# knights-lab/BURST

Hardware: AMD Instinct MI355X
Metric: aligned reads/sec (node), 100-bp synthetic reads @0.98 id vs RefSeq stand-in .edx/.acx (DB15), -m BEST; 1 GPU (higher is better)
Workload: dtype u32 bit-vectors (u8 edit distances)

## Files before the change

burst_amd/csrc/bhip_align.hip:

```cpp
#include "bhip_handle.h"
#include "bhip_pf_select.h"

__global__ void k_hit_count(const BhipHit *__restrict__ hits, uint32_t n, const uint32_t *__restrict__ n_dev, uint32_t *__restrict__ cnt, uint32_t *__restrict__ rank) {
	if (n_dev) n = *n_dev < n ? *n_dev : n;
	for (uint32_t i = blockIdx.x * blockDim.x + threadIdx.x; i < n; i += gridDim.x * blockDim.x) rank[i] = atomicAdd(&cnt[hits[i].q], 1u);
}
__global__ void k_hit_scatter(const BhipHit *__restrict__ in, uint32_t n, const uint32_t *__restrict__ n_dev, const uint32_t *__restrict__ off, const uint32_t *__restrict__ rank,
                              BhipHit *__restrict__ out, const uint32_t *__restrict__ qmap) {
	if (n_dev) n = *n_dev < n ? *n_dev : n;
	for (uint32_t i = blockIdx.x * blockDim.x + threadIdx.x; i < n; i += gridDim.x * blockDim.x) {
		BhipHit h = in[i];
		const uint32_t dst = off[h.q] + rank[i];
		if (qmap) h.q = qmap[h.q];
		out[dst] = h;
	}
}
__global__ void k_junk_adjust_raw(BhipRawHit *__restrict__ raw, const uint32_t *__restrict__ n_raw_dev, uint32_t raw_cap, const uint8_t *__restrict__ nx) {
	uint32_t n = *n_raw_dev;
	if (n > raw_cap) n = raw_cap;
	for (uint32_t i = blockIdx.x * blockDim.x + threadIdx.x; i < n; i += gridDim.x * blockDim.x) { const uint32_t x = nx[raw[i].q]; raw[i].ed += x; raw[i].m += x; }
}
__global__ void k_junk_adjust_best(uint32_t *__restrict__ best, const uint8_t *__restrict__ nx_six, uint32_t s0, uint32_t s1) {
	for (uint32_t s = s0 + blockIdx.x * blockDim.x + threadIdx.x; s < s1; s += gridDim.x * blockDim.x)
		if (nx_six[s] && best[s] != 0xFFFFFFFFu) best[s] += nx_six[s];
// ... 325 lines not shown
	HIPCHK(hipEventRecord(ev[SPAN_START], st));
	const uint64_t full = (n_thr + 255) / 256;
	const uint32_t grid = (uint32_t)(ahead && h->opt_seed_ahead_blocks > 0 ? std::min<uint64_t>(full, (uint64_t)h->n_cu * (uint64_t)h->opt_seed_ahead_blocks) : full);
	hipLaunchKernelGGL(k_seed_ranges, dim3(grid), dim3(256), 0, st,
		junk ? S->qcodes_s.as<uint8_t>() : S->qcodes.as<uint8_t>(), junk ? S->qoff_s.as<uint64_t>() : S->qoff.as<uint64_t>(), d_qlist, n_list,
		h->acx_view(), h->K, S->plan.as<uint32_t>(), W16, L->ranges_c[cls].as<uint2>(), L->hdr_c[cls].as<uint2>(),
		junk ? S->qpack_s.as<uint32_t>() : S->qpack.as<uint32_t>(), (S->st_maxlen + 7) / 8, junk ? S->qemac_s.as<uint16_t>() : S->qemac.as<uint16_t>(), qm.as<uint4>(), S->st_has_six ? S->qsix.as<uint32_t>() : nullptr,
		seed_min_need_for(h, mean_words, W16), (uint32_t)h->opt_seed_drop_len, h->alt);
	HIPCHK(hipGetLastError());
	HIPCHK(hipEventRecord(ev[SPAN_DONE], st));
	L->qmeta_seq[S->seq & 1][cls] = S->seq + 1;
	L->seeded_ok[cls] = true; L->seeded_seq[cls] = S->seq; L->seeded_n[cls] = n_list; L->seeded_W16[cls] = W16;
	return 0;
}

static bhip_pf_kernel_t pf_kernel(const BhipPfChoice &c, int big) {
	if (c.legacy) return bhip_legacy_pf_kernel ? bhip_legacy_pf_kernel(c.kind, big ? 11 : c.htb, big ? 4 : c.rb, c.cw_mode, big) : nullptr;
	if (c.kind == BHIP_PF_CQ) return c.cw_mode == 0 ? (big ? k_prefilter_cq<0, 1> : k_prefilter_cq<0, 0>) : (big ? k_prefilter_cq<1, 1> : k_prefilter_cq<1, 0>);
	return big ? k_prefilter_cw<2, 1> : k_prefilter_cw<2, 0>;
}

static int launch_prefilter_mask(Handle *h, Lane *L, hipStream_t st, int cls, const uint32_t *d_qlist, uint32_t n_list, uint32_t maxwords, uint32_t *n_tasks_dev,
                                 uint32_t *n_cand_dev, Counters *dc, int algo, int prune) {
	int rc;
	PfOverflow ov;
	if ((rc = ov.begin(L, dc, st, n_list, true))) return rc;
	const uint32_t W16 = seed_row_words(maxwords);
	const double mean_words = n_list ? (double)L->seed_words[cls] / (double)n_list : (double)maxwords;
	if (!(L->seeded_ok[cls] && L->seeded_seq[cls] == h->cur->seq && L->seeded_n[cls] == n_list && L->seeded_W16[cls] == W16))
		if ((rc = launch_seed(h, L, st, h->cur, cls, d_qlist, n_list, maxwords, mean_words))) return rc;
	const BhipPfChoice c = bhip_pf_choose(algo, h->opt_pf_cw, h->opt_pf_table, h->opt_pf_rb, W16, mean_words * h->acx_wmean);
	const bool filter = c.kind != BHIP_PF_MASK, cw = c.kind == BHIP_PF_CW || c.kind == BHIP_PF_CQ;
	const bhip_pf_kernel_t fp = filter ? pf_kernel(c, 0) : nullptr, fp2 = filter && c.two_pass ? pf_kernel(c, 1) : nullptr;
	if (filter && (!fp || (c.two_pass && !fp2)))
		return fail(BHIP_E_ARG, "option prefilter_cw = %d selects a superseded prefilter kernel that is not part of libburst_hip.so (tests: libburst_hip_legacy.so is loaded first)", h->opt_pf_cw);
	hipFuncAttributes fa;
	const void *fn = filter ? (const void *)fp : c.htb == 9 ? (const void *)k_prefilter_mask<9> : c.htb == 10 ? (const void *)k_prefilter_mask<10> : (const void *)k_prefilter_mask<11>;
	const uint32_t fit = std::min<uint32_t>(cw ? 32u : 12u, blocks_per_cu(fn, 64u, 0, &fa));
	if (getenv("BHIP_DEBUG")) {
		if (cw) fprintf(stderr, "[bhip] prefilter kernel: %s, slot mode %d, %zu B LDS, %d VGPRs -> %u blocks per CU\n", c.kind == BHIP_PF_CQ ? "four queries per wave, streams by the whole wave" : "one query per wave", c.cw_mode, fa.sharedSizeBytes, fa.numRegs, fit);
		else fprintf(stderr, "[bhip] prefilter kernel: table 2^%d, %d record blocks in registers, %zu B LDS, %d VGPRs -> %u blocks per CU\n", c.htb, c.rb, fa.sharedSizeBytes, fa.numRegs, fit);
	}
	const uint32_t waves = h->opt_pf_waves ? std::min<uint32_t>((uint32_t)h->opt_pf_waves, fit) : fit;
	const uint32_t grid = std::min<uint32_t>(c.kind == BHIP_PF_CW ? n_list : (n_list + 3) / 4, (uint32_t)h->n_cu * waves);
	HIPCHK(hipEventRecord(L->ev_pf[cls][PF_HASH_START], st));
	const uint32_t *fb_dense = ov.fb1, *n_fb_dense = ov.n_fb1;
	if (filter) {
		auto launch = [&](bhip_pf_kernel_t k, uint32_t g, uint32_t *fb, uint32_t *n_fb, const uint32_t *sel, const uint32_t *n_sel) {
			hipLaunchKernelGGL(k, dim3(g), dim3(64), 0, st, L->ranges_c[cls].as<uint2>(), L->hdr_c[cls].as<uint2>(), W16, n_list,
				h->acx_view().rec, h->bad.as<uint32_t>(), h->n_bad,
				h->clump_len.as<uint32_t>(), h->tot_refs, L->tasks.as<uint2>(), n_tasks_dev, (uint32_t)L->task_cap, &dc->ent_read,
				fb, n_fb, &dc->unit_sum, &dc->col_sum, &dc->qlen_sum, &dc->surv_sum,
				L->tasks2.as<uint2>(), &dc->n_tasks2_cls[cls], prune, sel, n_sel, c.kind == BHIP_PF_CF ? h->opt_pf_bytes : 0);
		};
		launch(fp, grid, ov.fb1, ov.n_fb1, nullptr, nullptr);
		if (c.two_pass) {
			HIPCHK(hipGetLastError());
			const uint32_t g2 = (uint32_t)h->n_cu * (c.kind == BHIP_PF_CQ ? std::min<uint32_t>(4u, blocks_per_cu((const void *)fp2, 64u, 0)) : 1u);
			launch(fp2, g2, ov.fb2, ov.n_fb2, ov.fb1, ov.n_fb1);
			fb_dense = ov.fb2; n_fb_dense = ov.n_fb2;
		}
	} else {
		dispatch_int(HtbList{}, c.htb, [&](auto htb) {
			hipLaunchKernelGGL(k_prefilter_mask<decltype(htb)::value>, dim3(grid), dim3(64), 0, st, L->ranges_c[cls].as<uint2>(), L->hdr_c[cls].as<uint2>(), W16, n_list,
				h->acx_view().rec, h->bad.as<uint32_t>(), h->n_bad,
				h->clump_len.as<uint32_t>(), h->tot_refs, L->tasks.as<uint2>(), n_tasks_dev, (uint32_t)L->task_cap, &dc->ent_read,
				ov.fb1, ov.n_fb1, &dc->unit_sum, &dc->col_sum, &dc->qlen_sum, L->cand.as<uint2>(), n_cand_dev, (uint32_t)L->cand_cap);
		});
	}
	HIPCHK(hipGetLastError());
	HIPCHK(hipEventRecord(L->ev_pf[cls][PF_HASH_DONE], st));
	++L->pf_launches;
	L->pf_algo_used = c.kind;
	return launch_dense_fallback(h, L, st, d_qlist, n_list, h->bad.as<uint32_t>(), h->n_bad, L->cand.as<uint2>(), nullptr, n_cand_dev, (uint32_t)L->cand_cap, dc, fb_dense, n_fb_dense);
}

static int lane_reserve_work(Lane *L) {
	int rc;
	if ((rc = L->cand.reserve(L->cand_cap * sizeof(uint2))) || (rc = L->raw.reserve(L->raw_cap * sizeof(BhipRawHit))) || (rc = L->wide.reserve(L->raw_cap * sizeof(uint32_t))) ||
	    (rc = L->rs_lists.reserve(L->raw_cap * sizeof(uint32_t) * 10)) || (rc = L->scratch.reserve(L->scratch_cap * sizeof(uint32_t))) || (rc = L->wins.reserve(L->win_cap * sizeof(BhipWin))) ||
	    (rc = L->tasks.reserve(L->task_cap * sizeof(uint2))) || (rc = L->tasks2.reserve(L->task_cap * sizeof(uint2))) || (rc = L->tasks2k.reserve(L->task_cap * sizeof(uint2))) ||
	    (rc = L->wins2.reserve(L->win_cap * sizeof(BhipWin)))) return rc;
	return 0;
}
extern "C" int bhip_reserve(void *handle, uint32_t n_entries, uint32_t max_len) { return bhip_reserve_symbols(handle, n_entries, max_len, 0); }
extern "C" int bhip_reserve_symbols(void *handle, uint32_t n_entries, uint32_t max_len, uint64_t total_symbols) {
	Handle *h = (Handle *)handle;
	if (!h) return fail(BHIP_E_ARG, "null handle");
	if (!n_entries) return BHIP_OK;
	if (!max_len || max_len > BHIP_MAX_QLEN) max_len = BHIP_MAX_QLEN;
	HIPCHK(hipSetDevice(h->device));
	int rc;
	if (getenv("BHIP_DEBUG")) { size_t f_ = 0, t_ = 0; if (hipMemGetInfo(&f_, &t_) == hipSuccess) fprintf(stderr, "[bhip] reserve for %u entries of up to %u symbols: %.2f GB of the device's %.2f free\n", n_entries, max_len, f_ / 1e9, t_ / 1e9); }
	const size_t n = n_entries, nb = total_symbols ? (size_t)std::min<uint64_t>(total_symbols + 64, (uint64_t)n * max_len) : n * max_len, qw = (max_len + 7) / 8;
	const size_t cw = (size_t)class_words(class_of_len(max_len), max_len);
	const size_t peq_words = total_symbols ? std::min<size_t>(n * cw, 2 * (nb / 32 + n)) : n * cw;
	for (StageSlot &S : h->slots) {
		if ((rc = slot_init(&S))) return rc;
		if ((rc = S.qcodes4.reserve(nb / 2 + 128)) || (rc = S.qcodes.reserve(nb + 128)) || (rc = S.qoff.reserve((n + 1) * 8)) || (rc = S.qemac.reserve((n + 1) * 2)) ||
		    (rc = S.qsix.reserve((n + 1) * 4)) || (rc = S.qrc.reserve(n + 1)) || (rc = S.qflags.reserve(n + 1)) || (rc = S.qmap.reserve((n + 1) * 4)) ||
		    (rc = S.off_raw.reserve((n + 8) * 8)) || (rc = S.plan.reserve(n * 4 + 16)) || (rc = S.qpack.reserve(n * qw * 4 + 64)) || (rc = S.key.reserve(n + 16)) ||
		    (rc = S.key_sorted.reserve(n + 16)) || (rc = S.idx.reserve(n * 4 + 16)) || (rc = S.idx_sorted.reserve(n * 4 + 16))) return rc;
		size_t tb = 0;
		HIPCHK(hipcub::DeviceRadixSort::SortPairs(nullptr, tb, S.key.as<uint8_t>(), S.key_sorted.as<uint8_t>(), S.idx.as<uint32_t>(), S.idx_sorted.as<uint32_t>(), (int)n, 0, 8, h->stage_stream));
		if ((rc = S.sort_tmp.reserve(tb + 16))) return rc;
	}
	if (getenv("BHIP_DEBUG")) { size_t f_ = 0, t_ = 0; if (hipMemGetInfo(&f_, &t_) == hipSuccess) fprintf(stderr, "[bhip] ... staging slots reserved: %.2f GB free\n", f_ / 1e9); }
	if ((rc = ensure_lanes(h, 1))) return rc;
	Lane *L = h->lanes[0];
	lane_capacity_floor(h, L, n);
	const int cls = class_of_len(max_len);
	if ((rc = lane_reserve_work(L)) || (rc = L->peq.reserve(peq_words * 16 * 4)) || (rc = L->peqp.reserve(n * 16 * 6 * 4)) ||
	    (rc = L->peq_alt.reserve(peq_words * 16 * 4)) || (rc = L->peqp_alt.reserve(n * 16 * 6 * 4)) ||
	    (rc = L->fb_list.reserve(n * 8 + 64)) || (rc = L->ranges_c[cls].reserve(n * 16 * 8 + 16)) || (rc = L->hdr_c[cls].reserve(n * 8 + 16))) return rc;
	if (h->n_order) { if ((rc = h->best_key.reserve((n + 1) * 8)) || (rc = h->sort_idx.reserve(std::max<size_t>((size_t)h->out_cap, n + 1) * 4))) return rc; if (!h->nsel_pinned) HIPCHK(hipHostMalloc((void **)&h->nsel_pinned, 64, hipHostMallocDefault)); }
	if ((rc = h->best.reserve((n + 1) * 4)) || (rc = h->out.reserve(h->out_cap * sizeof(BhipHit))) || (rc = h->shared_ctr.reserve(sizeof(SharedCtr))) ||
	    (rc = h->sort_idx.reserve(h->out_cap * 4)) || (rc = h->sort_keys.reserve((n + 1) * 4)) || (rc = h->sort_keys2.reserve((n + 1) * 4)) ||
	    (rc = h->out_sorted.reserve(h->out_cap * sizeof(BhipHit))) || (rc = h->out_sorted2.reserve(h->out_cap * sizeof(BhipHit)))) return rc;
	{
		size_t tb = 0;
		HIPCHK(hipcub::DeviceScan::ExclusiveSum(nullptr, tb, h->sort_keys.as<uint32_t>(), h->sort_keys2.as<uint32_t>(), (int)(n + 1), h->stream));
		if ((rc = h->sort_tmp.reserve(tb))) return rc;
	}
	if (getenv("BHIP_DEBUG")) { size_t f_ = 0, t_ = 0; if (hipMemGetInfo(&f_, &t_) == hipSuccess) fprintf(stderr, "[bhip] ... lane and record buffers reserved: %.2f GB free\n", f_ / 1e9); }
	if (!h->copy_stream) { HIPCHK(hipStreamCreateWithFlags(&h->copy_stream, hipStreamNonBlocking)); HIPCHK(hipEventCreateWithFlags(&h->ev_sorted, hipEventDisableTiming));
		for (auto &e : h->ev_copied) HIPCHK(hipEventCreateWithFlags(&e, hipEventDisableTiming)); }
	{
		const uint32_t nw = std::min<uint32_t>(n_entries, 1u << 17), len = std::min<uint32_t>(max_len, 100u);
		const size_t nb_w = (size_t)nw * len + 16;
		uint8_t *pin = nullptr;
		const size_t bytes = nb_w + nb_w / 2 + 16 + ((size_t)nw + 1) * 8 + (size_t)nw * 2 + 64 + (size_t)nw * 4 * sizeof(BhipHit);
		HIPCHK(hipHostMalloc((void **)&pin, bytes, hipHostMallocPortable));
		uint8_t *codes = pin, *codes4 = pin + nb_w;
		uint64_t *off = (uint64_t *)(pin + ((nb_w + nb_w / 2 + 16 + 7) & ~(size_t)7));
		uint16_t *emac = (uint16_t *)(off + nw + 1);
		BhipHit *hbuf = (BhipHit *)(((uintptr_t)(emac + nw) + 63) & ~(uintptr_t)63);
		uint64_t x = 88172645463325252ull;
		for (size_t i = 0; i < nb_w; ++i) { x ^= x << 13; x ^= x >> 7; x ^= x << 17; codes[i] = (uint8_t)(1 + (x & 3)); }
		for (size_t i = 0; i < nb_w / 2; ++i) codes4[i] = (uint8_t)(codes[2 * i] | codes[2 * i + 1] << 4);
		for (uint32_t i = 0; i <= nw; ++i) off[i] = (uint64_t)i * len;
		for (uint32_t i = 0; i < nw; ++i) emac[i] = (uint16_t)(len / 40);
		BhipQuerySpan sp;
		memset(&sp, 0, sizeof sp);
		sp.codes = codes; sp.codes4 = codes4; sp.off = off; sp.emac = emac; sp.n = nw;
		uint64_t n_out = 0;
		const int async = h->opt_async_d2h;
		h->opt_async_d2h = 1;
		for (StageSlot &S : h->slots) { S.state = 0; S.st_valid = false; }
		rc = 0;
		for (int rep = 0; rep < 4 && !rc; ++rep) {
			rc = bhip_stage_spans(h, &sp, 1, nw, len);
			if (!rc) rc = bhip_align_staged(h, 0, hbuf, (uint64_t)nw * 4, &n_out);
		}
		(void)bhip_sync_hits(h);
		{
			const size_t big = std::min<size_t>(64u << 20, std::min(h->out_sorted.cap, h->out_sorted2.cap));
			void *tmp = nullptr;
			if (big && hipHostMalloc(&tmp, 2 * big, hipHostMallocPortable) == hipSuccess) {
				(void)hipMemcpyAsync(tmp, h->out_sorted.p, big, hipMemcpyDeviceToHost, h->copy_stream);
				(void)hipMemcpyAsync((char *)tmp + big, h->out_sorted2.p, big, hipMemcpyDeviceToHost, h->copy_stream);
				(void)hipMemcpyAsync(tmp, h->out_sorted.p, big, hipMemcpyDeviceToHost, h->copy_stream);
				(void)hipStreamSynchronize(h->copy_stream);
				(void)hipMemcpyAsync(h->out_sorted.p, tmp, big, hipMemcpyHostToDevice, h->stage_stream);
				(void)hipMemcpyAsync(h->out_sorted2.p, (char *)tmp + big, big, hipMemcpyHostToDevice, h->stage_stream);
				(void)hipMemcpyAsync(h->out_sorted.p, tmp, big, hipMemcpyHostToDevice, h->stage_stream);
				(void)hipStreamSynchronize(h->stage_stream);
				const size_t piece = big / 16;
				if (piece) {
					for (int i = 0; i < 12; ++i) (void)hipMemcpyAsync((char *)h->out_sorted.p + (size_t)i * piece, (char *)tmp + (size_t)i * piece, piece, hipMemcpyHostToDevice, h->stage_stream);
					(void)hipMemcpyAsync((char *)tmp + big, h->out_sorted2.p, big, hipMemcpyDeviceToHost, h->copy_stream);
					(void)hipStreamSynchronize(h->copy_stream);
					(void)hipStreamSynchronize(h->stage_stream);
				}
				(void)hipHostFree(tmp);
			}
			(void)hipGetLastError();
		}
		h->opt_async_d2h = async;
		for (StageSlot &S : h->slots) { S.state = 0; S.st_valid = false; S.spans.clear(); }
		h->res_valid = false;
		(void)hipHostFree(pin);
		if (rc) return rc;
	}
	return BHIP_OK;
}
enum { STEP_REDO = 1 };
struct BatchCall {
	StageSlot *slot = nullptr;
	int mode = 0;
	int all_hits = 0;
	bool sel_best = false;
	BhipHit *hits = nullptr; uint64_t cap = 0; uint64_t *n_hits = nullptr;
	uint32_t n_q = 0, n_shared = 0, nl = 0;
	uint32_t band_rows = 0, qw = 0, rw = 0;
	SharedCtr hsc = {};
	uint32_t n_deliver = 0;
	bool sorted_ahead = false; int o_ahead = 0;
	size_t tmp_bytes = 0;
	std::chrono::steady_clock::time_point t0; double t_host[4] = {0, 0, 0, 0};
	void mark(int i) { t_host[i] = std::chrono::duration<double, std::milli>(std::chrono::steady_clock::now() - t0).count(); }
};

static int enqueue_class(Handle *h, Lane *L, int cls, int all_hits) {
	int rc;
	hipStream_t pf = h->pf_stream, sw = h->sweep_stream, po = h->post_stream;
	Counters *dc = L->counters.as<Counters>();
	const uint32_t n_pf = L->npf[cls], n_ex = L->nex[cls], n_list = n_pf + n_ex;
	const uint32_t grid_my = (uint32_t)h->n_cu * (uint32_t)h->opt_sweep_blocks;
	const uint32_t grid_task = (uint32_t)h->n_cu * 4u * (uint32_t)h->opt_sweep_blocks * (uint32_t)h->opt_oversub;
	const int NW = class_words(cls, L->maxlen);
	const uint32_t *qlist = L->qlist[cls];
	hipEvent_t *ce = L->ev_cls[cls];
	if (L->launches) { HIPCHK(hipStreamWaitEvent(pf, L->ev_rs[RS_START], 0)); HIPCHK(hipStreamWaitEvent(sw, L->ev_rs[RS_START], 0)); }
	const int NWP = class_prefix_words(h, L->maxE[cls], NW);
	HIPCHK(hipEventRecord(ce[CE_START], sw));
	L->peq_ahead[cls] = false;
	if (L->alt_ok && L->alt_seq == h->cur->seq && L->alt_cls == cls && L->alt_n == n_list && L->alt_nwp == NWP && !L->launches) {
		std::swap(L->peq, L->peq_alt); std::swap(L->peqp, L->peqp_alt);
		std::swap(L->ev_peq_cur[SPAN_START], L->ev_peq_alt[SPAN_START]); std::swap(L->ev_peq_cur[SPAN_DONE], L->ev_peq_alt[SPAN_DONE]);
		L->alt_ok = false; L->peq_ahead[cls] = true;
	} else if ((rc = launch_peq(h, sw, h->cur, qlist, n_list, NW, NWP, L->peq, L->peqp))) return rc;
	L->prefix_words = (uint32_t)NWP;
	HIPCHK(hipEventRecord(ce[CE_PEQ_DONE], sw));
	HIPCHK(hipEventRecord(ce[CE_PF_START], pf));
	const bool masked = NWP && n_pf && h->has_masks && h->opt_lane_masks;
	const int pf_algo = bhip_pf_algo(h->opt_pf_algo, L->pf_algo);
	const int prune = masked && !all_hits && h->opt_prune && n_list < (1u << 24) && pf_algo == 0;
	if (n_pf) {
		if (masked) { if ((rc = launch_prefilter_mask(h, L, pf, cls, qlist, n_pf, L->maxwords[cls], &dc->n_tasks_cls[cls], &dc->n_cand_cls[cls], dc, pf_algo, prune))) return rc; }
		else if ((rc = launch_prefilter(h, L, pf, qlist, n_pf, L->cand.as<uint2>(), nullptr, (uint32_t)L->cand_cap, true, &dc->n_cand_cls[cls], dc))) return rc;
	}
	const uint4 *qmeta_cls = (masked && L->qmeta_seq[h->cur->seq & 1][cls] == h->cur->seq + 1) ? L->qmeta_c[h->cur->seq & 1][cls].as<uint4>() : nullptr;
	L->masked = masked;
	L->pf_masked[cls] = masked && n_pf;
	HIPCHK(hipEventRecord(ce[CE_PF_DONE], pf));
	HIPCHK(hipStreamWaitEvent(sw, ce[CE_PF_DONE], 0));
	HIPCHK(hipEventRecord(ce[CE_SWEEP_START], sw));
	if (n_pf) {
		if (masked) launch_prefix_task(h, L, sw, NWP, grid_task, L->tasks.as<uint2>(), &dc->n_tasks_cls[cls], qlist, L->wins.as<BhipWin>(), &dc->n_wins_cls[cls], dc, qmeta_cls);
		if (NWP) launch_prefix(h, L, sw, NWP, masked ? std::min<uint32_t>(grid_my, (uint32_t)h->n_cu) : grid_my, L->cand.as<uint2>(), &dc->n_cand_cls[cls], L->cand_cap, 0, qlist, &dc->n_wins_cls[cls], dc);
		else launch_myers(h, L, sw, NW, grid_my, L->cand.as<uint2>(), &dc->n_cand_cls[cls], L->cand_cap, 0, qlist, L->raw.as<BhipRawHit>(),
			&dc->n_raw, (uint32_t)L->raw_cap, h->best.as<uint32_t>(), nullptr, dc);
		HIPCHK(hipGetLastError());
		++L->launches;
	}
	HIPCHK(hipEventRecord(ce[CE_SWEEP_PF_DONE], sw));
	if (n_ex) {
		const uint64_t np = (uint64_t)n_ex * h->n_clumps;
		const uint32_t g = (uint32_t)std::min<uint64_t>((np + 15) / 16, grid_my);
		if (NWP) launch_prefix(h, L, sw, NWP, g, nullptr, nullptr, np, n_pf, qlist, &dc->n_wins_cls[cls], dc);
		else launch_myers(h, L, sw, NW, g, nullptr, nullptr, np, n_pf, qlist, L->raw.as<BhipRawHit>(), &dc->n_raw, (uint32_t)L->raw_cap,
			h->best.as<uint32_t>(), nullptr, dc);
		HIPCHK(hipGetLastError());
		++L->launches;
		L->n_pairs_ex += np;
	}
	HIPCHK(hipEventRecord(ce[CE_SWEEP_EX_DONE], sw));
	HIPCHK(hipStreamWaitEvent(po, ce[CE_SWEEP_EX_DONE], 0));
	if (NWP) { launch_window(h, L, po, cls, NWP, grid_my, L->wins.as<BhipWin>(), &dc->n_wins_cls[cls], dc); HIPCHK(hipGetLastError()); }
	L->pruned[cls] = masked && prune && n_pf;
	if (L->pruned[cls]) {
		HIPCHK(hipEventRecord(L->ev_ph[cls][PH_WIN_DONE], po));
		HIPCHK(hipStreamWaitEvent(sw, L->ev_ph[cls][PH_WIN_DONE], 0));
		hipLaunchKernelGGL(k_task_filter, dim3((uint32_t)h->n_cu * 8), dim3(256), 0, sw, L->tasks2.as<uint2>(), &dc->n_tasks2_cls[cls], (uint32_t)L->task_cap, qlist,
			six_or_null(h), h->best.as<uint32_t>(), L->tasks2k.as<uint2>(), &dc->n_tasks2k_cls[cls]);
		launch_prefix_task(h, L, sw, NWP, grid_task, L->tasks2k.as<uint2>(), &dc->n_tasks2k_cls[cls], qlist, L->wins2.as<BhipWin>(), &dc->n_wins2_cls[cls], dc, qmeta_cls);
		HIPCHK(hipGetLastError());
		HIPCHK(hipEventRecord(L->ev_ph[cls][PH_SWEEP2_DONE], sw));
		HIPCHK(hipStreamWaitEvent(po, L->ev_ph[cls][PH_SWEEP2_DONE], 0));
		launch_window(h, L, po, cls, NWP, grid_my, L->wins2.as<BhipWin>(), &dc->n_wins2_cls[cls], dc);
		HIPCHK(hipGetLastError());
	}
	HIPCHK(hipEventRecord(ce[CE_WIN_DONE], po));
	HIPCHK(hipEventRecord(L->ev_rs[RS_START], po));
	return 0;
}

static int enqueue_rescore(Handle *h, Lane *L, const BatchCall &b) {
	hipStream_t po = h->post_stream;
	Counters *dc = L->counters.as<Counters>();
	SharedCtr *sc = h->shared_ctr.as<SharedCtr>();
	const RefArgs R = ref_args(h);
	HIPCHK(hipEventRecord(L->ev_rs[RS_START], po));
	if (h->cur->st_has_junk) {
		const uint32_t nl_ = h->cur->st_lanes, nsh_ = h->cur->st_nshared;
		uint32_t li_ = 0;
		for (uint32_t l = 0; l < nl_; ++l) if (h->lanes[l] == L) li_ = l;
		const uint32_t s0 = (uint32_t)(((uint64_t)li_ * nsh_ + nl_ - 1) / nl_), s1 = (uint32_t)(((uint64_t)(li_ + 1) * nsh_ + nl_ - 1) / nl_);
		hipLaunchKernelGGL(k_junk_adjust_raw, dim3((uint32_t)h->n_cu * 4), dim3(256), 0, po, L->raw.as<BhipRawHit>(), &dc->n_raw, (uint32_t)L->raw_cap, h->cur->nx.as<uint8_t>());
		if (s1 > s0) hipLaunchKernelGGL(k_junk_adjust_best, dim3(std::min<uint32_t>((s1 - s0 + 255) / 256, (uint32_t)h->n_cu * 4)), dim3(256), 0, po, h->best.as<uint32_t>(), h->cur->nx_six.as<uint8_t>(), s0, s1);
		HIPCHK(hipGetLastError());
	}
	const uint32_t qw_g = (h->cur->st_maxlen + 7) / 8;
	hipLaunchKernelGGL(k_rescore_classify, dim3((uint32_t)h->n_cu * 8), dim3(256), 0, po, L->raw.as<BhipRawHit>(), &dc->n_raw, (uint32_t)L->raw_cap,
		h->best.as<uint32_t>(), b.all_hits, h->cur->qoff.as<uint64_t>(), six_or_null(h), rc_or_null(h),
		R.len, h->out.as<BhipHit>(), &sc->n_out, (uint32_t)h->out_cap, L->rs_lists.as<uint32_t>(), dc->n_rs, L->wide.as<uint32_t>(), &dc->n_wide,
		b.band_rows, h->opt_rescore_reg);
	HIPCHK(hipGetLastError());
	if (h->opt_rescore_reg) {
		for_each_int(SetList{}, [&](auto set) {
			constexpr int SET = decltype(set)::value;
			const uint32_t grid = (uint32_t)h->n_cu * std::min<uint32_t>(32u, blocks_per_cu((const void *)k_rescore_reg<SET>, 64, 0)) * (uint32_t)h->opt_oversub;
			hipLaunchKernelGGL(k_rescore_reg<SET>, dim3(grid), dim3(64), 0, po, L->raw.as<BhipRawHit>(), L->rs_lists.as<uint32_t>(), dc->n_rs, (uint32_t)L->raw_cap,
				h->cur->qoff.as<uint64_t>(), rc_or_null(h), h->cur->qpack.as<uint32_t>(), qw_g,
				R.bytes(), R.off, R.len, h->lut.as<uint8_t>(), h->out.as<BhipHit>(), &sc->n_out, (uint32_t)h->out_cap, &sc->err);
		});
		HIPCHK(hipGetLastError());
	}
	const uint32_t grid_rs = (uint32_t)h->n_cu * (h->opt_rescore_reg ? 4 : 16);
	const size_t lds_rs = (size_t)(b.band_rows + 1 + b.qw + b.rw) * 256;
	hipLaunchKernelGGL(k_rescore<false>, dim3(grid_rs), dim3(64), lds_rs, po, L->raw.as<BhipRawHit>(), &dc->n_raw, (uint32_t)L->raw_cap,
		L->rs_lists.as<uint32_t>() + (size_t)9 * L->raw_cap, &dc->n_rs[9], h->best.as<uint32_t>(), b.all_hits, h->cur->qcodes.as<uint8_t>(), h->cur->qoff.as<uint64_t>(),
		six_or_null(h), rc_or_null(h), R.bytes(), R.off, R.len, h->lut.as<uint8_t>(), h->out.as<BhipHit>(), &sc->n_out, (uint32_t)h->out_cap, L->wide.as<uint32_t>(),
		&dc->n_wide, (uint32_t *)nullptr, &dc->scratch_used, 0ull, &sc->err, b.qw ? h->cur->qpack.as<uint32_t>() : nullptr, b.band_rows, b.qw, b.rw);
	HIPCHK(hipGetLastError());
	HIPCHK(hipEventRecord(L->ev_rs[RS_DONE], po));
	HIPCHK(hipMemcpyAsync(L->hc_pinned, dc, sizeof(Counters), hipMemcpyDeviceToHost, po));
	return 0;
}

static int enqueue_lane(Handle *h, Lane *L, const BatchCall &b) {
	int rc;
	if ((rc = lane_reserve_work(L))) return rc;
	HIPCHK(hipMemsetAsync(L->counters.p, 0, sizeof(Counters), h->pf_stream));
	L->launches = 0; L->prefix_words = 0; L->n_pairs_ex = 0; L->pf_launches = 0; L->fb_dirty = false;
	for (int c = 0; c < kNumClasses; ++c) { L->pf_masked[c] = false; L->pruned[c] = false; }
	for (int cls = 0; cls < kNumClasses; ++cls) if (L->npf[cls] + L->nex[cls]) if ((rc = enqueue_class(h, L, cls, b.all_hits))) return rc;
	return enqueue_rescore(h, L, b);
}

static void seed_next_batch(Handle *h, StageSlot *cur, hipEvent_t cur_done) {
	if (!h->opt_seed_ahead || !h->has_acx || !h->has_masks || !h->opt_lane_masks || h->opt_host_routing) return;
	StageSlot *N = nullptr;
	for (StageSlot &S : h->slots) if (&S != cur && S.state == 1 && (!N || S.seq < N->seq)) N = &S;
	if (!N || !N->st_nq) return;
	if (!N->resolved) {
		for (;;) {
			const hipError_t e = hipEventQuery(N->ev_done);
			if (e == hipSuccess) break;
			if (e != hipErrorNotReady) { (void)hipGetLastError(); return; }
			if (hipEventQuery(cur_done) != hipErrorNotReady) { (void)hipGetLastError(); return; }
			std::this_thread::yield();
		}
		(void)hipGetLastError();
		const BhipStageInfo &I = *N->info_pinned;
		if (I.err || I.junk) return;
		if (resolve_slot(h, N)) return;
	}
	if (N->st_has_junk || ensure_lanes(h, N->st_lanes)) return;
	for (uint32_t l = 0; l < N->st_lanes && l < h->lanes.size(); ++l) {
		Lane *L = h->lanes[l];
		for (int cls = 0; cls < kNumClasses; ++cls) {
			const uint32_t n_pf = N->npf[l][cls];
			if (!n_pf || !class_prefix_words(h, N->maxE[l][cls], class_words(cls, N->maxlen_lane[l]))) continue;
			if (L->seeded_ok[cls] && L->seeded_seq[cls] == N->seq) continue;
			if (launch_seed(h, L, h->pf_stream, N, cls, N->idx_sorted.as<uint32_t>() + N->qlist_off[l][cls], n_pf, N->maxwords[l][cls], (double)N->seed_words[l][cls] / (double)n_pf, true)) { (void)hipGetLastError(); return; }
		}
		int only = -1, n_cls = 0;
		for (int cls = 0; cls < kNumClasses; ++cls) if (N->npf[l][cls] + N->nex[l][cls]) { only = cls; ++n_cls; }
		if (n_cls == 1 && !(L->alt_ok && L->alt_seq == N->seq)) {
			const uint32_t n_list = N->npf[l][only] + N->nex[l][only];
			const int NW = class_words(only, N->maxlen_lane[l]), NWP = class_prefix_words(h, N->maxE[l][only], NW);
			L->alt_ok = false;
			if (hipEventRecord(L->ev_peq_alt[SPAN_START], h->pf_stream) != hipSuccess ||
			    launch_peq(h, h->pf_stream, N, N->idx_sorted.as<uint32_t>() + N->qlist_off[l][only], n_list, NW, NWP, L->peq_alt, L->peqp_alt, (uint32_t)h->opt_peq_ahead_blocks) ||
			    hipEventRecord(L->ev_peq_alt[SPAN_DONE], h->pf_stream) != hipSuccess) { (void)hipGetLastError(); return; }
			L->alt_ok = true; L->alt_seq = N->seq; L->alt_cls = only; L->alt_nwp = NWP; L->alt_n = n_list;
		}
	}
}

extern "C" int bhip_set_enqueued_hook(void *handle, void (*fn)(void *), void *ctx) {
	Handle *h = (Handle *)handle;
	if (!h) return fail(BHIP_E_ARG, "null handle");
	h->enqueued_hook = fn; h->enqueued_ctx = ctx;
	return BHIP_OK;
}

static bool grow_cap(uint64_t &cap, uint64_t seen, bool eighth, int lane, const char *what) {
	if (seen <= cap) return false;
	const uint64_t to = seen + (eighth ? seen / 8 : 0) + 1024;
	if (getenv("BHIP_DEBUG")) {
		if (lane >= 0) fprintf(stderr, "[bhip] redo: lane %d %s %llu -> %llu\n", lane, what, (unsigned long long)cap, (unsigned long long)to);
		else fprintf(stderr, "[bhip] redo: %s %llu -> %llu\n", what, (unsigned long long)cap, (unsigned long long)to);
	}
	cap = to;
	return true;
}

static int pick_batch(Handle *h, BatchCall &b) {
	StageSlot *slot = nullptr;
	for (StageSlot &S : h->slots) if (S.state == 1 && (!slot || S.seq < slot->seq)) slot = &S;
	if (!slot) for (StageSlot &S : h->slots) if (S.state == 2 && (!slot || S.seq > slot->seq)) slot = &S;
	if (!slot) return fail(BHIP_E_ARG, "no staged queries (call bhip_stage_queries first)");
	{ int rcs = resolve_slot(h, slot); if (rcs) { slot->state = 0; return rcs; } }
	apply_slot(h, slot);
	b.slot = slot; b.n_q = h->cur->st_nq; b.n_shared = h->cur->st_nshared; b.nl = h->cur->st_lanes;
	return BHIP_OK;
}
static int plan_batch(Handle *h, BatchCall &b) {
	b.band_rows = std::min<uint32_t>(BHIP_RESCORE_WMAX, 2 * h->cur->st_maxE + 1 + 9);
	b.qw = (h->cur->st_maxlen + 7) / 8; b.rw = (h->cur->st_maxlen + b.band_rows + 24) / 8 + 2;
	if ((size_t)(b.band_rows + 1 + b.qw + b.rw) * 256 > 40 * 1024) { b.qw = 0; b.rw = 0; }
	if (!b.sel_best) return BHIP_OK;
	int rc;
	if ((rc = h->best_key.reserve((size_t)(b.n_q + 1) * 8)) || (rc = h->sort_idx.reserve(std::max<size_t>((size_t)h->out_cap, (size_t)b.n_q + 1) * 4))) return rc;
	if (!h->nsel_pinned) HIPCHK(hipHostMalloc((void **)&h->nsel_pinned, 64, hipHostMallocDefault));
	return BHIP_OK;
}
static bool records_resident(const Handle *h, const BatchCall &b) { return h->res_valid && h->res_seq == b.slot->seq && h->res_all_hits == b.mode; }
static void take_resident(Handle *h, BatchCall &b) {
	b.hsc.n_out = h->res_n_raw; b.hsc.err = 0; h->stats = h->res_stats; b.n_deliver = h->res_n; *b.n_hits = b.n_deliver; b.sorted_ahead = false;
}

static int plan_scan(Handle *h, BatchCall &b, hipStream_t st) {
	b.tmp_bytes = 0;
	HIPCHK(hipcub::DeviceScan::ExclusiveSum(nullptr, b.tmp_bytes, h->sort_keys.as<uint32_t>(), h->sort_keys2.as<uint32_t>(), (int)(b.n_q + 1), st));
	return h->sort_tmp.reserve(b.tmp_bytes);
}
static int enqueue_grouping(Handle *h, const BatchCall &b, hipStream_t st, uint32_t n_host, const uint32_t *n_dev, DBuf &sorted) {
	uint32_t *cnt = h->sort_keys.as<uint32_t>(), *off = h->sort_keys2.as<uint32_t>(), *rank = h->sort_idx.as<uint32_t>();
	const uint32_t n_q = b.n_q, g = (uint32_t)h->n_cu * 8;
	const uint32_t *qmap = h->cur->has_qmap ? h->cur->qmap.as<uint32_t>() : (const uint32_t *)nullptr;
	size_t tmp_bytes = b.tmp_bytes;
	if (b.sel_best) {
		hipLaunchKernelGGL(k_best_key, dim3(g), dim3(256), 0, st, h->out.as<BhipHit>(), n_host, n_dev, h->ref_order.as<uint32_t>(), cnt, h->best_key.as<unsigned long long>());
		hipLaunchKernelGGL(k_best_flag, dim3(std::min<uint32_t>((n_q + 256) / 256, g)), dim3(256), 0, st, cnt, n_q, rank);
		HIPCHK(hipcub::DeviceScan::ExclusiveSum(h->sort_tmp.p, tmp_bytes, rank, off, (int)(n_q + 1), st));
		hipLaunchKernelGGL(k_best_emit, dim3(g), dim3(256), 0, st, h->out.as<BhipHit>(), n_host, n_dev, h->ref_order.as<uint32_t>(), cnt, h->best_key.as<unsigned long long>(), off, sorted.as<BhipHit>(), qmap);
		HIPCHK(hipGetLastError());
		HIPCHK(hipMemcpyAsync(h->nsel_pinned, off + n_q, 4, hipMemcpyDeviceToHost, st));
		return 0;
	}
	HIPCHK(hipcub::DeviceScan::ExclusiveSum(h->sort_tmp.p, tmp_bytes, cnt, off, (int)(n_q + 1), st));
	hipLaunchKernelGGL(k_hit_scatter, dim3(g), dim3(256), 0, st, h->out.as<BhipHit>(), n_host, n_dev, off, rank, sorted.as<BhipHit>(), qmap);
	hipLaunchKernelGGL(k_hit_fix, dim3(std::min<uint32_t>((n_q + 255) / 256, (uint32_t)h->n_cu * 8)), dim3(256), 0, st, sorted.as<BhipHit>(), off, cnt, n_q, h->sort_scratch.as<BhipHit>(), (uint32_t)(h->sort_scratch.cap / sizeof(BhipHit)));
	HIPCHK(hipGetLastError());
	return 0;
}
static int enqueue_grouping_ahead(Handle *h, BatchCall &b) {
	int rc;
	b.o_ahead = (h->opt_async_d2h && b.hits) ? (h->out_idx ^ 1) : 0;
	DBuf &sorted = b.o_ahead ? h->out_sorted2 : h->out_sorted;
	if ((rc = h->sort_idx.reserve((size_t)h->out_cap * 4)) || (rc = h->sort_keys.reserve((size_t)(b.n_q + 1) * 4)) || (rc = h->sort_keys2.reserve((size_t)(b.n_q + 1) * 4)) ||
	    (rc = sorted.reserve((size_t)h->out_cap * sizeof(BhipHit))) || (rc = h->sort_scratch.reserve((size_t)h->out_cap * sizeof(BhipHit)))) return rc;
	if ((rc = plan_scan(h, b, h->post_stream))) return rc;
	if (h->copy_pending[b.o_ahead]) HIPCHK(hipStreamWaitEvent(h->post_stream, h->ev_copied[b.o_ahead], 0));
	HIPCHK(hipEventRecord(h->ev[EV_GROUP_START], h->post_stream));
	if ((rc = enqueue_grouping(h, b, h->post_stream, (uint32_t)h->out_cap, &h->shared_ctr.as<SharedCtr>()->n_out, sorted))) return rc;
	HIPCHK(hipEventRecord(h->ev[EV_GROUP_DONE], h->post_stream));
	b.sorted_ahead = true;
	return BHIP_OK;
}

static int enqueue_chain(Handle *h, BatchCall &b, int attempt) {
	int rc;
	const uint32_t n_q = b.n_q;
	b.sorted_ahead = false;
	if ((rc = h->best.reserve((size_t)(b.n_shared + 1) * 4)) || (rc = h->out.reserve(h->out_cap * sizeof(BhipHit))) || (rc = h->shared_ctr.reserve(sizeof(SharedCtr)))) return rc;
	HIPCHK(hipEventRecord(h->ev[EV_BEGIN], h->stream));
	HIPCHK(hipMemsetAsync(h->best.p, 0xFF, (size_t)b.n_shared * 4, h->stream));
	HIPCHK(hipMemsetAsync(h->shared_ctr.p, 0, 2 * sizeof(uint32_t), h->stream));
	if ((rc = h->sort_idx.reserve((size_t)h->out_cap * 4)) || (rc = h->sort_keys.reserve((size_t)(n_q + 1) * 4))) return rc;
	HIPCHK(hipMemsetAsync(h->sort_keys.p, 0, (size_t)(n_q + 1) * 4, h->stream));
	if (b.sel_best) HIPCHK(hipMemsetAsync(h->best_key.p, 0xFF, (size_t)(n_q + 1) * 8, h->stream));
	hipLaunchKernelGGL(k_set_rank_ptrs, dim3(1), dim3(1), 0, h->stream, h->shared_ctr.as<SharedCtr>(), h->sort_keys.as<uint32_t>(), h->sort_idx.as<uint32_t>());
	HIPCHK(hipEventRecord(h->ev[EV_RESET_DONE], h->stream));
	HIPCHK(hipStreamWaitEvent(h->sweep_stream, h->ev[EV_RESET_DONE], 0));
	HIPCHK(hipStreamWaitEvent(h->post_stream, h->ev[EV_RESET_DONE], 0));
	for (uint32_t l = 0; l < b.nl; ++l) if (h->lanes[l]->n_entries) if ((rc = enqueue_lane(h, h->lanes[l], b))) return rc;
	HIPCHK(hipEventRecord(h->ev[EV_PF_DONE], h->pf_stream));
	if ((rc = enqueue_grouping_ahead(h, b))) return rc;
	if (!h->hsc_pinned) HIPCHK(hipHostMalloc((void **)&h->hsc_pinned, sizeof(SharedCtr), hipHostMallocDefault));
	HIPCHK(hipMemcpyAsync(h->hsc_pinned, h->shared_ctr.p, 2 * sizeof(uint32_t), hipMemcpyDeviceToHost, h->post_stream));
	HIPCHK(hipEventRecord(h->ev[EV_CHAIN_DONE], h->post_stream));
	seed_next_batch(h, b.slot, h->ev[EV_CHAIN_DONE]);
	if (h->enqueued_hook && attempt == 0) h->enqueued_hook(h->enqueued_ctx);
	return BHIP_OK;
}
static int wait_chain(Handle *h, const BatchCall &b) {
	HIPCHK(hipEventSynchronize(h->ev[EV_PF_DONE]));
	HIPCHK(hipStreamSynchronize(h->sweep_stream));
	HIPCHK(hipStreamSynchronize(h->post_stream));
	for (uint32_t l = 0; l < b.nl; ++l) if (h->lanes[l]->n_entries) h->lanes[l]->hc = *h->lanes[l]->hc_pinned;
	return BHIP_OK;
}
static void adapt_prefilter_algo(Handle *h, const BatchCall &b) {
	for (uint32_t l = 0; l < b.nl; ++l) {
		Lane *L = h->lanes[l];
		const bool cq_min_only = !b.all_hits && h->opt_pf_cw == 2 && L->pf_algo_used == 3;
		if (L->n_entries && L->pf_algo == 0 && !cq_min_only && L->hc.ent_read > 100000 && (double)L->hc.surv_sum > (b.all_hits ? 0.20 : 0.50) * (double)L->hc.ent_read) L->pf_algo = 1;
	}
}
static void print_chain_counters(const Handle *h, const BatchCall &b) {
	for (uint32_t l = 0; l < b.nl; ++l) {
		const Lane *L = h->lanes[l];
		if (!L->n_entries) continue;
		fprintf(stderr, "[bhip] lane %u: %llu list records, %llu survived the counting filter, next prefilter algorithm %d\n", l, (unsigned long long)L->hc.ent_read, (unsigned long long)L->hc.surv_sum, L->pf_algo);
		for (int cls = 0; cls < kNumClasses; ++cls) if (L->npf[cls] + L->nex[cls])
			fprintf(stderr, "[bhip] lane %u class NW=%d: prefiltered %u exhaustive %u maxE %u maxwords %u | tasks %u + deferred %u (kept %u) clump pairs %u windows %u + %u | fallback queries(last class) %u raw %u\n",
				l, kClasses[cls], L->npf[cls], L->nex[cls], L->maxE[cls], L->maxwords[cls], L->hc.n_tasks_cls[cls], L->hc.n_tasks2_cls[cls], L->hc.n_tasks2k_cls[cls], L->hc.n_cand_cls[cls], L->hc.n_wins_cls[cls], L->hc.n_wins2_cls[cls], L->hc.n_fb, L->hc.n_raw);
		if (L->hc.n_fb) fprintf(stderr, "[bhip] lane %u: %u queries overflowed the first prefilter pass, %u the second (dense fallback)\n", l, L->hc.n_fb, L->hc.n_fb2);
		const uint32_t *rs = L->hc.n_rs;
		fprintf(stderr, "[bhip] lane %u: re-scorer bands 4:%u 6:%u 8:%u 12:%u 16:%u 24:%u 32:%u 40:%u 48:%u lds:%u scratch:%u\n",
			l, rs[0], rs[1], rs[2], rs[3], rs[4], rs[5], rs[6], rs[7], rs[8], rs[9], L->hc.n_wide);
	}
}
static int grow_lane_capacities(Handle *h, const BatchCall &b) {
	bool redo = false;
	for (uint32_t l = 0; l < b.nl; ++l) {
		Lane *L = h->lanes[l];
		if (!L->n_entries) continue;
		const Counters &c = L->hc;
		for (int cls = 0; cls < kNumClasses; ++cls) {
			redo |= grow_cap(L->cand_cap, c.n_cand_cls[cls], true, (int)l, "cand");
			redo |= grow_cap(L->task_cap, c.n_tasks_cls[cls], true, (int)l, "tasks");
			redo |= grow_cap(L->task_cap, c.n_tasks2_cls[cls], true, (int)l, "tasks");
			redo |= grow_cap(L->win_cap, c.n_wins2_cls[cls], true, (int)l, "wins");
			redo |= grow_cap(L->win_cap, c.n_wins_cls[cls], true, (int)l, "wins");
		}
		redo |= grow_cap(L->raw_cap, c.n_raw, true, (int)l, "raw");
	}
	return redo ? STEP_REDO : BHIP_OK;
}
static int rescore_wide_bands(Handle *h, BatchCall &b) {
	bool redo = false;
	const RefArgs R = ref_args(h);
	SharedCtr *sc = h->shared_ctr.as<SharedCtr>();
	for (uint32_t l = 0; l < b.nl; ++l) {
		Lane *L = h->lanes[l];
		if (!L->n_entries || !L->hc.n_wide) continue;
		b.sorted_ahead = false;
		if (getenv("BHIP_DEBUG")) fprintf(stderr, "[bhip] lane %u: n_wide %u hits through the global-scratch re-scorer\n", l, L->hc.n_wide);
		Counters *dc = L->counters.as<Counters>();
		hipLaunchKernelGGL(k_rescore<true>, dim3(std::min<uint32_t>((L->hc.n_wide + 63) / 64, (uint32_t)h->n_cu * 16)), dim3(64), 256, h->post_stream,
			L->raw.as<BhipRawHit>(), &dc->n_raw, (uint32_t)L->raw_cap, L->wide.as<uint32_t>(), &dc->n_wide, h->best.as<uint32_t>(), b.all_hits,
			h->cur->qcodes.as<uint8_t>(), h->cur->qoff.as<uint64_t>(), six_or_null(h), rc_or_null(h),
			R.bytes(), R.off, R.len, h->lut.as<uint8_t>(), h->out.as<BhipHit>(),
			&sc->n_out, (uint32_t)h->out_cap, (uint32_t *)nullptr, (uint32_t *)nullptr, L->scratch.as<uint32_t>(), &dc->scratch_used,
			(unsigned long long)L->scratch_cap, &sc->err, (const uint32_t *)nullptr, 0u, 0u, 0u);
		HIPCHK(hipGetLastError());
		HIPCHK(hipMemcpyAsync(&L->hc, dc, sizeof(Counters), hipMemcpyDeviceToHost, h->post_stream));
		HIPCHK(hipStreamSynchronize(h->post_stream));
		redo |= grow_cap(L->scratch_cap, L->hc.scratch_used, false, (int)l, "scratch");
	}
	if (b.sorted_ahead) b.hsc = *h->hsc_pinned;
	else HIPCHK(hipMemcpy(&b.hsc, h->shared_ctr.p, 2 * sizeof(uint32_t), hipMemcpyDeviceToHost));
	return redo || (b.hsc.err & 2u) ? STEP_REDO : BHIP_OK;
}
static int check_shared_counters(Handle *h, BatchCall &b) {
	if (b.hsc.err & 1u) return fail(BHIP_E_RESCORE, "re-scoring could not reproduce a hit found by the edit-distance kernel (a query starting with a symbol outside the alphabet? the reference stops here as well: CRITICAL ERROR: Truncation within known good path, burst.c:812-816)");
	if (grow_cap(h->out_cap, b.hsc.n_out, true, -1, "out")) return STEP_REDO;
	b.n_deliver = b.sel_best ? (b.sorted_ahead ? *h->nsel_pinned : std::min<uint32_t>(b.hsc.n_out, b.n_q)) : b.hsc.n_out;
	*b.n_hits = b.n_deliver;
	h->last_n_out = 0;
	return BHIP_OK;
}
static void collect_stats(Handle *h, const BatchCall &b) {
	BhipStats &S = h->stats;
	S.n_queries = b.n_q; S.n_hits = b.n_deliver;
	uint64_t qlen_sum = 0;
	for (uint32_t l = 0; l < b.nl; ++l) {
		Lane *L = h->lanes[l];
		if (!L->n_entries) continue;
		const Counters &c = L->hc;
		S.n_pairs += L->n_pairs_ex + c.unit_sum; S.n_columns += c.col_sum; S.n_task_columns += c.tcol_sum; S.n_raw_hits += c.n_raw; S.acx_entries_read += c.ent_read;
		S.myers_launches += L->launches; S.prefilter_launches += L->pf_launches; if (L->pf_launches) S.prefilter_algo = (uint32_t)L->pf_algo_used; S.n_window_columns += c.wcol_sum; qlen_sum += c.qlen_sum;
		if (L->prefix_words) S.prefix_words = L->prefix_words;
		for (int cls = 0; cls < kNumClasses; ++cls) {
			S.n_pairs += c.n_cand_cls[cls]; S.n_windows += c.n_wins_cls[cls] + c.n_wins2_cls[cls]; S.n_lane_tasks += c.n_tasks_cls[cls] + c.n_tasks2k_cls[cls];
			if (!(L->npf[cls] + L->nex[cls])) continue;
			hipEvent_t *ce = L->ev_cls[cls];
			S.ms_peq += L->peq_ahead[cls] ? ev_ms(L->ev_peq_cur[SPAN_START], L->ev_peq_cur[SPAN_DONE]) : ev_ms(ce[CE_START], ce[CE_PEQ_DONE]);
			if (L->npf[cls]) S.ms_prefilter += ev_ms(ce[CE_PF_START], ce[CE_PF_DONE]);
			if (L->npf[cls] && L->pf_masked[cls]) {
				hipEvent_t *es = L->ev_seed[h->cur->seq & 1][cls];
				S.ms_seed += ev_ms(es[SPAN_START], es[SPAN_DONE]); S.ms_prefilter_hash += ev_ms(L->ev_pf[cls][PF_HASH_START], L->ev_pf[cls][PF_HASH_DONE]); S.n_seed_words += L->seed_words[cls];
			}
			float sweep = ev_ms(ce[CE_SWEEP_START], ce[CE_SWEEP_EX_DONE]), win = ev_ms(ce[CE_SWEEP_EX_DONE], ce[CE_WIN_DONE]);
			if (L->pruned[cls]) { const float second = ev_ms(L->ev_ph[cls][PH_WIN_DONE], L->ev_ph[cls][PH_SWEEP2_DONE]); sweep += second; win -= second; }
			S.ms_myers += sweep + win;
			if (L->prefix_words) { S.ms_myers_prefix += sweep; S.ms_myers_window += win; }
		}
		S.ms_rescore += ev_ms(L->ev_rs[RS_START], L->ev_rs[RS_DONE]);
	}
	S.bytes_algorithmic = 8ull * S.n_columns + qlen_sum / 2 + 192ull * S.n_pairs;
	h->res_valid = true; h->res_seq = b.slot->seq; h->res_all_hits = b.mode; h->res_n = b.n_deliver; h->res_n_raw = b.hsc.n_out; h->res_stats = h->stats;
}
static int run_chain(Handle *h, BatchCall &b, int attempt) {
	int rc;
	if ((rc = enqueue_chain(h, b, attempt)) || (rc = wait_chain(h, b))) return rc;
	adapt_prefilter_algo(h, b);
	if (getenv("BHIP_DEBUG")) print_chain_counters(h, b);
	if ((rc = grow_lane_capacities(h, b)) || (rc = rescore_wide_bands(h, b)) || (rc = check_shared_counters(h, b))) return rc;
	collect_stats(h, b);
	return BHIP_OK;
}

static int group_late(Handle *h, BatchCall &b, int o, DBuf &sorted) {
	int rc;
	const uint32_t n = b.hsc.n_out, n_q = b.n_q;
	if (h->copy_pending[o]) { HIPCHK(hipEventSynchronize(h->ev_copied[o])); h->copy_pending[o] = false; }
	if ((rc = sorted.reserve((size_t)n * sizeof(BhipHit))) || (rc = h->sort_scratch.reserve((size_t)n * sizeof(BhipHit)))) return rc;
	uint32_t *cnt = h->sort_keys.as<uint32_t>(), *rank = h->sort_idx.as<uint32_t>();
	HIPCHK(hipMemsetAsync(cnt, 0, (size_t)(n_q + 1) * 4, h->stream));
	if (b.sel_best) HIPCHK(hipMemsetAsync(h->best_key.p, 0xFF, (size_t)(n_q + 1) * 8, h->stream));
	b.mark(0);
	hipLaunchKernelGGL(k_hit_count, dim3(std::min<uint32_t>((n + 255) / 256, (uint32_t)h->n_cu * 8)), dim3(256), 0, h->stream, h->out.as<BhipHit>(), n, (const uint32_t *)nullptr, cnt, rank);
// ... 240 lines not shown
```

burst_amd/csrc/bhip_handle.h:

```cpp
#ifndef BHIP_HANDLE_H
#define BHIP_HANDLE_H
#include <hip/hip_runtime.h>
#include <hipcub/hipcub.hpp>
#include <string>
#include <stdint.h>
#include <stdio.h>
#include <stdarg.h>
#include <stdlib.h>
#include <string.h>
#include <algorithm>
#include <vector>
#include <mutex>
#include <atomic>
#include <chrono>
#include <thread>
#include "burst_hip.h"
#include "bhip_internal.h"

__global__ void k_acx_offsets(const uint32_t *, uint64_t, int, uint32_t *, unsigned long long *);
__global__ void k_acx_lines(const uint32_t *, uint64_t, int, unsigned long long *, uint4 *);
__global__ void k_acx_decode(const uint8_t *, const unsigned long long *, const uint32_t *, BhipAcxView, uint64_t, int, uint32_t, uint32_t *, uint32_t *);
__global__ void k_transpose_refs(const uint8_t *, const uint64_t *, const uint32_t *, const uint64_t *, uint32_t, uint4 *);
__global__ void k_build_peq(const uint8_t *, const uint64_t *, const uint32_t *, uint32_t, int, int, BhipMatchMask, uint32_t *, const uint32_t *, uint32_t, uint32_t);
template <bool LDS_CNT> __global__ void k_prefilter(const uint8_t *, const uint64_t *, const uint16_t *, const uint32_t *, uint32_t,
	BhipAcxView, int, uint32_t, uint32_t *, const uint32_t *, uint32_t, uint2 *, uint32_t *, uint32_t *, uint32_t,
	unsigned long long *, const uint32_t *, const uint32_t *, const uint32_t *);
__global__ void k_prefilter_hash(const uint8_t *, const uint64_t *, const uint16_t *, const uint32_t *, uint32_t, BhipAcxView, int,
	const uint32_t *, uint32_t, uint2 *, uint32_t *, uint32_t *, uint32_t, unsigned long long *, const uint32_t *, uint32_t *, uint32_t *);
template <typename CNT> __global__ void k_prefilter_wave(const uint8_t *, const uint64_t *, const uint16_t *, const uint32_t *, uint32_t,
	BhipAcxView, int, uint32_t, const uint32_t *, uint32_t, uint2 *, uint32_t *, uint32_t *, uint32_t, unsigned long long *, const uint32_t *,
	const uint32_t *, const uint32_t *);
template <int NW> __global__ void k_myers(const uint2 *, const uint32_t *, uint64_t, uint32_t, uint32_t, const uint32_t *, const uint32_t *,
	const uint64_t *, const uint16_t *, const uint32_t *, const uint4 *, const uint64_t *, const uint32_t *, uint32_t,
	BhipRawHit *, uint32_t *, uint32_t, uint32_t *, uint8_t *, unsigned long long *, unsigned long long *);
__global__ void k_myers_long(const uint2 *, const uint32_t *, uint64_t, uint32_t, uint32_t, const uint32_t *, const uint32_t *,
	const uint64_t *, const uint16_t *, const uint32_t *, const uint4 *, const uint64_t *, const uint32_t *, uint32_t,
	BhipRawHit *, uint32_t *, uint32_t, uint32_t *, uint8_t *, unsigned long long *, unsigned long long *, uint32_t);
template <int NWP> __global__ void k_myers_prefix(const uint2 *, const uint32_t *, uint64_t, uint32_t, uint32_t, const uint32_t *, const uint32_t *,
	const uint64_t *, const uint16_t *, const uint4 *, const uint64_t *, const uint32_t *, uint32_t, BhipWin *, uint32_t *, uint32_t,
	unsigned long long *, unsigned long long *, uint32_t *, const uint32_t *);
template <int NW> __global__ void k_myers_window(const BhipWin *, const uint32_t *, uint32_t, int, int, const uint32_t *, const uint32_t *,
	const uint4 *, BhipRawHit *, uint32_t *, uint32_t, uint32_t *, unsigned long long *, const uint32_t *);
template <int BW> __global__ void k_myers_window_band(const BhipWin *, const uint32_t *, uint32_t, int, int, const uint32_t *, const uint32_t *,
	const uint4 *, BhipRawHit *, uint32_t *, uint32_t, uint32_t *, unsigned long long *, const uint32_t *);
__global__ void k_extract_kmers(const uint4 *, const uint64_t *, const uint32_t *, const uint64_t *, uint32_t, uint32_t, int, unsigned long long *, uint16_t *, uint32_t *);
__global__ void k_attach_masks(BhipAcxView, uint64_t, const unsigned long long *, const uint16_t *, uint32_t, const uint32_t *, uint32_t *, uint32_t, uint32_t);
template <int HTB> __global__ void k_prefilter_mask(const uint2 *, const uint2 *, uint32_t, uint32_t, const uint32_t *, const uint32_t *, uint32_t, const uint32_t *, uint32_t,
	uint2 *, uint32_t *, uint32_t, unsigned long long *, uint32_t *, uint32_t *, unsigned long long *, unsigned long long *, unsigned long long *,
	uint2 *, uint32_t *, uint32_t);
template <int MODE, int BIG> __global__ void k_prefilter_cq(const uint2 *, const uint2 *, uint32_t, uint32_t, const uint32_t *, const uint32_t *, uint32_t, const uint32_t *, uint32_t,
	uint2 *, uint32_t *, uint32_t, unsigned long long *, uint32_t *, uint32_t *, unsigned long long *, unsigned long long *, unsigned long long *, unsigned long long *,
	uint2 *, uint32_t *, int, const uint32_t *, const uint32_t *, int);
template <int MODE, int BIG> __global__ void k_prefilter_cw(const uint2 *, const uint2 *, uint32_t, uint32_t, const uint32_t *, const uint32_t *, uint32_t, const uint32_t *, uint32_t,
	uint2 *, uint32_t *, uint32_t, unsigned long long *, uint32_t *, uint32_t *, unsigned long long *, unsigned long long *, unsigned long long *, unsigned long long *,
	uint2 *, uint32_t *, int, const uint32_t *, const uint32_t *, int);
__global__ void k_task_filter(const uint2 *, const uint32_t *, uint32_t, const uint32_t *, const uint32_t *, const uint32_t *, uint2 *, uint32_t *);
__global__ void k_seed_ranges(const uint8_t *, const uint64_t *, const uint32_t *, uint32_t, BhipAcxView, int, const uint32_t *, uint32_t, uint2 *, uint2 *, const uint32_t *, uint32_t, const uint16_t *, uint4 *, const uint32_t *, uint32_t, uint32_t, BhipAlt);
template <int NWP> __global__ void k_myers_prefix_task(const uint2 *, const uint32_t *, uint32_t, const uint32_t *, const uint32_t *, const uint64_t *,
	const uint16_t *, const uint4 *, const uint64_t *, const uint32_t *, BhipWin *, uint32_t *, uint32_t, unsigned long long *, uint32_t *, const uint4 *, const uint32_t *);
template <bool WIDE> __global__ void k_rescore(const BhipRawHit *, const uint32_t *, uint32_t, const uint32_t *, const uint32_t *,
	const uint32_t *, int, const uint8_t *, const uint64_t *, const uint32_t *, const uint8_t *, const uint8_t *, const uint64_t *,
	const uint32_t *, const uint8_t *, BhipHit *, uint32_t *, uint32_t, uint32_t *, uint32_t *, uint32_t *, unsigned long long *,
	unsigned long long, uint32_t *, const uint32_t *, uint32_t, uint32_t, uint32_t);
__global__ void k_pack_queries(const uint8_t *, const uint64_t *, uint32_t, uint32_t, uint32_t *);
__global__ void k_unpack4(const uint8_t *, uint64_t, uint64_t, uint8_t *);
__global__ void k_unpack2(const uint8_t *, uint64_t, uint64_t, uint8_t *);
__global__ void k_span_fill(const uint64_t *, uint32_t, uint32_t, uint64_t, uint32_t, uint64_t *, uint32_t *, uint32_t *);
__global__ void k_route(const uint64_t *, const uint32_t *, uint32_t, const uint16_t *, const uint32_t *, const uint8_t *, uint32_t, uint32_t, uint32_t, int, int, int,
	uint32_t *, uint8_t *, uint32_t *, BhipStageInfo *, BhipAlt);
__global__ void k_rescore_classify(const BhipRawHit *, const uint32_t *, uint32_t, const uint32_t *, int, const uint64_t *, const uint32_t *, const uint8_t *,
	const uint32_t *, BhipHit *, uint32_t *, uint32_t, uint32_t *, uint32_t *, uint32_t *, uint32_t *, uint32_t, int);
template <int SET> __global__ void k_rescore_reg(const BhipRawHit *, const uint32_t *, const uint32_t *, uint32_t, const uint64_t *, const uint8_t *, const uint32_t *, uint32_t,
	const uint8_t *, const uint64_t *, const uint32_t *, const uint8_t *, BhipHit *, uint32_t *, uint32_t, uint32_t *);
int bhip_fail_msg(int code, const char *fmt, ...) __attribute__((format(printf, 2, 3)));
#define fail(...) bhip_fail_msg(__VA_ARGS__)
inline bool bhip_trace_sync() { static const bool on = getenv("BHIP_TRACE_SYNC") != nullptr; return on; }
#define HIPCHK(x) do { hipError_t e_ = (x); if (e_ != hipSuccess) \
	return fail(BHIP_E_DEVICE, "%s:%d %s: %s", __FILE__, __LINE__, #x, hipGetErrorString(e_)); \
	if (bhip_trace_sync()) { fprintf(stderr, "[bhip sync] %s:%d\n", __FILE__, __LINE__); (void)hipDeviceSynchronize(); } } while (0)

inline std::mutex &bhip_vmm_mutex() { static std::mutex m; return m; }
inline std::atomic<int> &bhip_vmm_peer_access() { static std::atomic<int> f(0); return f; }
struct DBuf {
	void *p = nullptr; size_t cap = 0;
	bool vmm = false; size_t va_size = 0; int vmm_device = 0;
	std::vector<hipMemGenericAllocationHandle_t> chunks;
	size_t n_mapped = 0;
	static constexpr size_t kChunk = 1ull << 30;
	static hipError_t malloc_patiently(void **q, size_t want) {
		hipError_t e = hipMalloc(q, want);
		if (e != hipErrorOutOfMemory) return e;
		(void)hipGetLastError();
		size_t last_free = 0, total = 0;
		(void)hipMemGetInfo(&last_free, &total);
		const bool dbg = getenv("BHIP_DEBUG") != nullptr;
		if (dbg) fprintf(stderr, "[bhip] hipMalloc(%zu) found no memory with %.2f GB reported free: waiting for memory that is on its way back\n", want, last_free / 1e9);
		for (int tries = 0; tries < 80; ++tries) {
			std::this_thread::sleep_for(std::chrono::milliseconds(100));
			e = hipMalloc(q, want);
			if (e != hipErrorOutOfMemory) { if (dbg) fprintf(stderr, "[bhip] ... there after %d ms\n", 100 * (tries + 1)); return e; }
			(void)hipGetLastError();
			if (dbg && tries % 10 == 9) { size_t f = 0; (void)hipMemGetInfo(&f, &total); fprintf(stderr, "[bhip] ... %d ms: %.2f GB reported free\n", 100 * (tries + 1), f / 1e9); }
		}
		return e;
	}
	static void poison(void *q, size_t n) {
		static const char *ev = getenv("BHIP_POISON");
		if (ev && q) { (void)hipMemset(q, atoi(ev) & 255, n); (void)hipDeviceSynchronize(); if (getenv("BHIP_DEBUG")) fprintf(stderr, "[bhip] buffer %p .. %p (%zu bytes)\n", q, (void *)((char *)q + n), n); }
	}
	int reserve(size_t bytes) {
		if (bytes <= cap) return 0;
		release();
		size_t want = bytes + bytes / 4 + 256;
		hipError_t e = malloc_patiently(&p, want);
		if (e != hipSuccess) { p = nullptr; return fail(BHIP_E_DEVICE, "hipMalloc(%zu): %s", want, hipGetErrorString(e)); }
		poison(p, want);
		cap = want; return 0;
	}
	int reserve_exact(size_t bytes) {
		if (bytes <= cap) return 0;
		release();
		hipError_t e = malloc_patiently(&p, bytes);
		if (e != hipSuccess) { p = nullptr; return fail(BHIP_E_DEVICE, "hipMalloc(%zu): %s", bytes, hipGetErrorString(e)); }
		poison(p, bytes);
		cap = bytes; return 0;
	}
	int reserve_growable(size_t max_bytes, int device) {
		release();
		std::lock_guard<std::mutex> lk(bhip_vmm_mutex());
		int ok = 0;
		if (hipDeviceGetAttribute(&ok, hipDeviceAttributeVirtualMemoryManagementSupported, device) != hipSuccess || !ok) { (void)hipGetLastError(); return 1; }
		const size_t sz = ((max_bytes + kChunk - 1) / kChunk + 1) * kChunk;
		if (hipMemAddressReserve(&p, sz, kChunk, nullptr, 0) != hipSuccess) { (void)hipGetLastError(); p = nullptr; return 1; }
		vmm = true; va_size = sz; vmm_device = device; cap = 0; n_mapped = 0;
		chunks.assign(sz / kChunk, nullptr);
		peers.clear();
		int n_dev = 0;
		if (bhip_vmm_peer_access().load() && hipGetDeviceCount(&n_dev) == hipSuccess) for (int d = 0; d < n_dev; ++d) { int can = 0; if (d != device && hipDeviceCanAccessPeer(&can, d, device) == hipSuccess && can) peers.push_back(d); }
		(void)hipGetLastError();
		return 0;
	}
	std::vector<int> peers;
	int map_chunks(size_t c0, size_t c1) {
		if (!vmm) return fail(BHIP_E_INTERNAL, "map_chunks on a fixed buffer");
		if (c1 > chunks.size()) return fail(BHIP_E_DEVICE, "record area: chunk %zu wanted, %zu reserved", c1, chunks.size());
		hipMemAllocationProp prop = {};
		prop.type = hipMemAllocationTypePinned; prop.location.type = hipMemLocationTypeDevice; prop.location.id = vmm_device;
		hipMemAccessDesc acc = {};
		acc.location.type = hipMemLocationTypeDevice; acc.location.id = vmm_device; acc.flags = hipMemAccessFlagsProtReadWrite;
		for (size_t c = c0; c < c1; ++c) {
			if (chunks[c]) continue;
			std::lock_guard<std::mutex> lk(bhip_vmm_mutex());
			hipMemGenericAllocationHandle_t hnd;
			hipError_t e = hipMemCreate(&hnd, kChunk, &prop, 0);
			if (e != hipSuccess) return fail(BHIP_E_DEVICE, "hipMemCreate(%zu) with %zu chunks mapped: %s", kChunk, n_mapped, hipGetErrorString(e));
			e = hipMemMap((char *)p + c * kChunk, kChunk, 0, hnd, 0);
			if (e == hipSuccess && !peers.empty()) {
				std::vector<hipMemAccessDesc> all(1 + peers.size(), acc);
				for (size_t k = 0; k < peers.size(); ++k) all[1 + k].location.id = peers[k];
				if (hipMemSetAccess((char *)p + c * kChunk, kChunk, all.data(), all.size()) != hipSuccess) { (void)hipGetLastError(); peers.clear(); }
			}
			if (e == hipSuccess && peers.empty()) e = hipMemSetAccess((char *)p + c * kChunk, kChunk, &acc, 1);
			if (e != hipSuccess) { (void)hipMemRelease(hnd); return fail(BHIP_E_DEVICE, "hipMemMap with %zu chunks mapped: %s", n_mapped, hipGetErrorString(e)); }
			chunks[c] = hnd; ++n_mapped;
		}
		size_t pre = cap / kChunk;
		while (pre < chunks.size() && chunks[pre]) ++pre;
		cap = pre * kChunk;
		return 0;
	}
	int grow_to(size_t bytes) {
		if (!vmm) return fail(BHIP_E_INTERNAL, "grow_to on a fixed buffer");
		if (bytes > va_size) return fail(BHIP_E_DEVICE, "record area: %zu bytes wanted, %zu reserved", bytes, va_size);
		return map_chunks(0, (bytes + kChunk - 1) / kChunk);
	}
	int grow_top_to(size_t bytes) {
		if (!vmm) return fail(BHIP_E_INTERNAL, "grow_top_to on a fixed buffer");
		if (bytes > va_size) return fail(BHIP_E_DEVICE, "record area: %zu bytes wanted at its top, %zu reserved", bytes, va_size);
		return map_chunks(chunks.size() - (bytes + kChunk - 1) / kChunk, chunks.size());
	}
	void shrink_to(size_t bytes) {
		if (!vmm) return;
		const size_t keep = (bytes + kChunk - 1) / kChunk;
		std::lock_guard<std::mutex> lk(bhip_vmm_mutex());
		for (size_t c = keep; c < chunks.size(); ++c) if (chunks[c]) {
			(void)hipMemUnmap((char *)p + c * kChunk, kChunk); (void)hipMemRelease(chunks[c]);
			chunks[c] = nullptr; --n_mapped;
		}
		if (cap > keep * kChunk) cap = keep * kChunk;
	}
	void release() {
		if (vmm) {
			std::lock_guard<std::mutex> lk(bhip_vmm_mutex());
			for (size_t c = 0; c < chunks.size(); ++c) if (chunks[c]) { (void)hipMemUnmap((char *)p + c * kChunk, kChunk); (void)hipMemRelease(chunks[c]); }
			chunks.clear(); n_mapped = 0;
			if (p) (void)hipMemAddressFree(p, va_size);
			vmm = false; va_size = 0;
		} else if (p) (void)hipFree(p);
		p = nullptr; cap = 0;
	}
	template <class T> T *as() const { return (T *)p; }
};

static const int kClasses[] = {2, 4, 6, 8, 10, 16, 32, 128};
static const int kNumClasses = BHIP_N_CLASSES;
static inline int class_of_len(uint32_t len) {
	for (int i = 0; i < kNumClasses - 1; ++i) if (len <= 32u * kClasses[i]) return i;
	return kNumClasses - 1;
}
static inline int class_words(int cls, uint32_t maxlen) { return cls == kNumClasses - 1 ? (int)((std::max<uint32_t>(maxlen, 1025u) + 31u) / 32u) : kClasses[cls]; }

struct Counters {
	uint32_t n_cand, n_raw, n_out, n_wide, err, pad0;
	uint32_t n_cand_cls[8];
	uint32_t n_wins_cls[8];
	uint32_t n_fb, n_fb2;
	uint32_t n_tasks_cls[8];
	uint32_t n_tasks2_cls[8];
	uint32_t n_tasks2k_cls[8];
	uint32_t n_wins2_cls[8];
	uint32_t n_rs[12];
	unsigned long long wcol_sum, tcol_sum, unit_sum;
	unsigned long long col_sum, qlen_sum, ent_read, scratch_used;
	unsigned long long surv_sum;
	uint32_t win_class_seen[4];
};

struct StageSlot {
	DBuf qcodes, qcodes4, qlen16, qoff, qemac, qsix, qrc, qflags, qmap, off_raw, plan, qpack, key, key_sorted, idx, idx_sorted, sort_tmp, info;
	DBuf qcodes_s, qoff_s, qemac_s, qpack_s, nx, nx_six;
	BhipStageInfo *info_pinned = nullptr;
	hipEvent_t ev_begin = nullptr, ev_done = nullptr, ev_copied = nullptr;
	int state = 0;
	uint64_t seq = 0;
	bool resolved = false;
	bool st_valid = false, st_has_six = false, st_has_rc = false, st_has_junk = false, has_flags = false, has_qmap = false;
	uint32_t st_nq = 0, st_nshared = 0, st_maxlen = 0, st_maxE = 0, st_lanes = 1;
	float st_ms_h2d = 0, st_ms_copy = 0, st_ms_route = 0;
	std::vector<BhipQuerySpan> spans;
	const uint32_t *six_explicit = nullptr;
	uint32_t npf[16][BHIP_N_CLASSES], nex[16][BHIP_N_CLASSES], maxE[16][BHIP_N_CLASSES], maxwords[16][BHIP_N_CLASSES], qlist_off[16][BHIP_N_CLASSES], maxlen_lane[16], n_entries_lane[16];
	uint64_t seed_words[16][BHIP_N_CLASSES];
	void release_all() {
		DBuf *b[] = {&qcodes, &qcodes4, &qlen16, &qoff, &qemac, &qsix, &qrc, &qflags, &qmap, &off_raw, &plan, &qpack, &key, &key_sorted, &idx, &idx_sorted,
			&sort_tmp, &info, &qcodes_s, &qoff_s, &qemac_s, &qpack_s, &nx, &nx_six};
		for (DBuf *x : b) x->release();
		if (info_pinned) { (void)hipHostFree(info_pinned); info_pinned = nullptr; }
		if (ev_begin) { (void)hipEventDestroy(ev_begin); ev_begin = nullptr; }
		if (ev_done) { (void)hipEventDestroy(ev_done); ev_done = nullptr; }
		if (ev_copied) { (void)hipEventDestroy(ev_copied); ev_copied = nullptr; }
	}
};

enum ClassEvent { CE_START, CE_PEQ_DONE, CE_PF_DONE, CE_SWEEP_PF_DONE, CE_SWEEP_EX_DONE, CE_WIN_DONE, CE_SWEEP_START, CE_PF_START, CE_COUNT };
enum { RS_START, RS_DONE };
enum { PH_WIN_DONE, PH_SWEEP2_DONE };
enum { PF_SEED_START, PF_HASH_START, PF_HASH_DONE };
enum { SPAN_START, SPAN_DONE };
enum { EV_BEGIN = 0, EV_RESET_DONE = 1, EV_KERNEL_DONE = 1, EV_PF_DONE = 2, EV_CHAIN_DONE = 3, EV_GROUP_START = 4, EV_GROUP_DONE = 5, EV_DELIVER_START = 8, EV_DELIVER_DONE = 9, EV_COUNT = 10 };

struct Lane {
	hipStream_t stream = nullptr;
	hipEvent_t ev_cls[kNumClasses][CE_COUNT];
	hipEvent_t ev_rs[2];
	hipEvent_t ev_ph[kNumClasses][2];
	hipEvent_t ev_pf[kNumClasses][3];
	uint64_t seed_words[kNumClasses] = {0};
	uint32_t pf_launches = 0;
	bool fb_dirty = false;
	bool pf_masked[kNumClasses] = {false};
	bool pruned[kNumClasses] = {false};
	int pf_algo_used = 0;
	int pf_algo = 0;
	const uint32_t *qlist[kNumClasses] = {nullptr};
	DBuf peq, peqp, cand, candcnt, wins, raw, wide, scratch, fb_list, gcnt, counters, tasks, tasks2, tasks2k, wins2, rs_lists;
	DBuf ranges_c[kNumClasses], hdr_c[kNumClasses];
	DBuf qmeta_c[2][kNumClasses];
	uint64_t qmeta_seq[2][kNumClasses] = {};
	bool seeded_ok[kNumClasses] = {false};
	uint64_t seeded_seq[kNumClasses] = {0};
	uint32_t seeded_n[kNumClasses] = {0}, seeded_W16[kNumClasses] = {0};
	hipEvent_t ev_seed[2][kNumClasses][2];
	DBuf peq_alt, peqp_alt;
	bool alt_ok = false; uint64_t alt_seq = 0; int alt_cls = 0, alt_nwp = 0; uint32_t alt_n = 0;
	hipEvent_t ev_peq_alt[2], ev_peq_cur[2];
	bool peq_ahead[kNumClasses] = {false};
	uint64_t task_cap = 1 << 20;
	uint64_t cand_cap = 1 << 18, raw_cap = 1 << 18, win_cap = 1 << 20, scratch_cap = 1 << 18;
	uint32_t npf[kNumClasses] = {0}, nex[kNumClasses] = {0}, maxE[kNumClasses] = {0}, maxwords[kNumClasses] = {0}, maxlen = 0, n_entries = 0;
	Counters *hc_pinned = nullptr;
	Counters hc;
	uint32_t launches = 0, prefix_words = 0;
	uint64_t n_pairs_ex = 0;
	bool masked = false;
};

struct SharedCtr { uint32_t n_out, err; uint32_t *cnt; uint32_t *rank; };
__global__ void k_set_rank_ptrs(SharedCtr *sc, uint32_t *cnt, uint32_t *rank);
struct Handle {
	int device = 0, n_cu = 0;
	char dev_name[256];
	uint64_t hbm = 0;
	hipStream_t stream = nullptr;
	hipStream_t pf_stream = nullptr;
	hipStream_t sweep_stream = nullptr;
	hipStream_t post_stream = nullptr;
	hipEvent_t ev[EV_COUNT];
	uint32_t n_clumps = 0, tot_refs = 0, max_clump_len = 0;
	DBuf ref_lane, ref_off, clump_len, lut;
	BhipMatchMask mm;
	BhipAlt alt;
	bool has_acx = false; int K = 0;
	int acx_z = 0;
	DBuf acx_lines, acx_rec, bad; uint32_t n_bad = 0; uint64_t n_ent = 0, acx_bias = 0;
	BhipAcxView acx_view() const {
		BhipAcxView v; v.lines = acx_lines.as<uint4>();
		v.rec = acx_rec.as<uint32_t>() - acx_bias; return v;
	}
	bool has_masks = false;
	int opt_lane_masks = 1;
	StageSlot slots[3];
	StageSlot *cur = &slots[0];
	uint64_t stage_seq = 0;
	hipStream_t stage_stream = nullptr;
	bool res_valid = false; uint64_t res_seq = 0; int res_all_hits = 0; uint32_t res_n = 0; BhipStats res_stats;
	int opt_host_routing = 0;
	DBuf best, out, shared_ctr, mins, pairs;
	DBuf ref_order, best_key; uint32_t n_order = 0;
	uint32_t *nsel_pinned = nullptr;
	uint32_t res_n_raw = 0;
	SharedCtr *hsc_pinned = nullptr;
	const uint8_t *s_codes() const { return cur->st_has_junk ? cur->qcodes_s.as<uint8_t>() : cur->qcodes.as<uint8_t>(); }
	const uint64_t *s_off() const { return cur->st_has_junk ? cur->qoff_s.as<uint64_t>() : cur->qoff.as<uint64_t>(); }
	const uint16_t *s_emac() const { return cur->st_has_junk ? cur->qemac_s.as<uint16_t>() : cur->qemac.as<uint16_t>(); }
	const uint32_t *s_pack() const { return cur->st_has_junk ? cur->qpack_s.as<uint32_t>() : cur->qpack.as<uint32_t>(); }
	DBuf sort_keys, sort_keys2, sort_idx, sort_tmp, out_sorted, out_sorted2, sort_scratch;
	uint64_t out_cap = 1 << 20;
	std::vector<uint32_t> h_clump_len;
	BhipStats stats;
	std::vector<Lane *> lanes;
	int opt_two_stage = 1;
	int opt_prefilter_stride = 0;
	int opt_lanes = 1;
	int opt_sweep_blocks = 8;
	uint32_t peq_rows = 16;
	int opt_oversub = 2;
	int opt_band_blocks = 0;
	int opt_no_band = 0;
	int opt_async_d2h = 0, out_idx = 0;
	hipStream_t copy_stream = nullptr;
	hipEvent_t ev_sorted = nullptr, ev_copied[2] = {nullptr, nullptr};
	bool copy_pending[2] = {false, false};
	void *reg_ptr[2] = {nullptr, nullptr}; size_t reg_bytes[2] = {0, 0};
	int last_out = 0;
	uint64_t last_n_out = 0;
	int opt_prune = 1;
	int opt_lane_min = 32768;
	int opt_rescore_reg = 1;
	int opt_pf_waves = 0;
	int opt_pf_algo = -1;
	int opt_pf_table = 0;
	int opt_pf_cw = 2;
	int opt_pf_bytes = 1;
	int opt_pf_rb = 0;
	int opt_seed_ahead = 1;
	int opt_seed_ahead_blocks = 2;
	int opt_peq_ahead_blocks = 16;
	void (*enqueued_hook)(void *) = nullptr; void *enqueued_ctx = nullptr;
	int opt_seed_min_need = -1;
	int opt_seed_drop_len = 8;
	double acx_wmean = 0.0;
	void *cov = nullptr;
	void *paths = nullptr;
	void *mates = nullptr;
	long long opt_cov_event_cap = 0;
};

static inline float ev_ms(hipEvent_t a, hipEvent_t b) { float ms = 0; (void)hipEventElapsedTime(&ms, a, b); return ms; }

int  ensure_lanes(Handle *h, uint32_t n);
uint32_t make_seed_plan(const uint8_t *s, uint32_t len, uint32_t E, uint32_t K, int stride_opt, const BhipAlt &A);
int  slot_init(StageSlot *S);
int  resolve_slot(Handle *h, StageSlot *S);
void apply_slot(Handle *h, StageSlot *S);
void lane_capacity_floor(Handle *h, Lane *L, uint64_t n);
int  bhip_load_accelerator(Handle *h, const uint32_t *acx_lens, const void *acx_lists, int acx_fmt, int K, const uint32_t *badlist, uint32_t n_bad);
int  bhip_build_accelerator(Handle *h, int K, int z);
void bhip_cov_release(Handle *h);
void bhip_paths_release(Handle *h);
void bhip_mates_release(Handle *h);
#endif
```

burst_amd/csrc/bhip_init.hip:

```cpp
#include "bhip_handle.h"

static thread_local char g_err[512] = "";

__global__ void k_ref_symbol_scan(const uint32_t *__restrict__ w, uint64_t n_words, uint32_t *__restrict__ flag) {
	uint32_t any = 0;
	for (uint64_t i = blockIdx.x * (uint64_t)blockDim.x + threadIdx.x; i < n_words; i += (uint64_t)gridDim.x * blockDim.x) {
		const uint32_t d = w[i];
		any |= (d | ((d << 1) & ((d << 2) | (d << 3)))) & 0x88888888u;
	}
	if (any) *flag = 1u;
}
int bhip_fail_msg(int code, const char *fmt, ...) {
	va_list ap; va_start(ap, fmt); vsnprintf(g_err, sizeof g_err, fmt, ap); va_end(ap);
	return code;
}

extern "C" const char *bhip_last_error(void) { return g_err; }
extern "C" int bhip_abi_version(void) { return BHIP_ABI_VERSION; }
std::atomic<int> &bhip_vmm_peer_access_flag() { return bhip_vmm_peer_access(); }

static void lane_destroy(Lane *L) {
	if (!L) return;
	DBuf *all[] = {&L->peq, &L->peqp, &L->cand, &L->candcnt, &L->wins, &L->raw, &L->wide, &L->scratch, &L->fb_list, &L->gcnt, &L->counters, &L->tasks, &L->tasks2, &L->tasks2k, &L->wins2, &L->rs_lists};
	for (DBuf *b : all) b->release();
	L->peq_alt.release(); L->peqp_alt.release();
	for (auto &e : L->ev_peq_alt) if (e) (void)hipEventDestroy(e);
	for (auto &e : L->ev_peq_cur) if (e) (void)hipEventDestroy(e);
	for (DBuf &b : L->ranges_c) b.release();
	for (DBuf &b : L->hdr_c) b.release();
	for (auto &pb : L->qmeta_c) for (DBuf &b : pb) b.release();
	for (auto &pe : L->ev_seed) for (auto &ce : pe) for (auto &e : ce) if (e) (void)hipEventDestroy(e);
	for (auto &ce : L->ev_cls) for (auto &e : ce) if (e) (void)hipEventDestroy(e);
	for (auto &e : L->ev_rs) if (e) (void)hipEventDestroy(e);
	for (auto &ce : L->ev_pf) for (auto &e : ce) if (e) (void)hipEventDestroy(e);
	for (auto &ce : L->ev_ph) for (auto &e : ce) if (e) (void)hipEventDestroy(e);
	if (L->hc_pinned) (void)hipHostFree(L->hc_pinned);
	delete L;
}

static int lane_create(Handle *h, Lane **out) {
	Lane *L = new Lane();
	memset(L->ev_cls, 0, sizeof L->ev_cls); memset(L->ev_rs, 0, sizeof L->ev_rs); memset(L->ev_pf, 0, sizeof L->ev_pf); memset(L->ev_ph, 0, sizeof L->ev_ph); memset(L->ev_seed, 0, sizeof L->ev_seed); memset(L->ev_peq_alt, 0, sizeof L->ev_peq_alt); memset(L->ev_peq_cur, 0, sizeof L->ev_peq_cur);
	L->stream = h->stream;
	for (auto &ce : L->ev_cls) for (auto &e : ce) if (hipEventCreate(&e) != hipSuccess) { lane_destroy(L); return fail(BHIP_E_DEVICE, "hipEventCreate failed"); }
	for (auto &e : L->ev_rs) if (hipEventCreate(&e) != hipSuccess) { lane_destroy(L); return fail(BHIP_E_DEVICE, "hipEventCreate failed"); }
	for (auto &ce : L->ev_pf) for (auto &e : ce) if (hipEventCreate(&e) != hipSuccess) { lane_destroy(L); return fail(BHIP_E_DEVICE, "hipEventCreate failed"); }
	for (auto &ce : L->ev_ph) for (auto &e : ce) if (hipEventCreate(&e) != hipSuccess) { lane_destroy(L); return fail(BHIP_E_DEVICE, "hipEventCreate failed"); }
	for (auto &pe : L->ev_seed) for (auto &ce : pe) for (auto &e : ce) if (hipEventCreate(&e) != hipSuccess) { lane_destroy(L); return fail(BHIP_E_DEVICE, "hipEventCreate failed"); }
	for (auto &e : L->ev_peq_alt) if (hipEventCreate(&e) != hipSuccess) { lane_destroy(L); return fail(BHIP_E_DEVICE, "hipEventCreate failed"); }
	for (auto &e : L->ev_peq_cur) if (hipEventCreate(&e) != hipSuccess) { lane_destroy(L); return fail(BHIP_E_DEVICE, "hipEventCreate failed"); }
	int rc = L->counters.reserve(sizeof(Counters));
	if (rc) { lane_destroy(L); return rc; }
	if (hipHostMalloc((void **)&L->hc_pinned, sizeof(Counters), hipHostMallocDefault) != hipSuccess) { lane_destroy(L); return fail(BHIP_E_DEVICE, "hipHostMalloc failed"); }
	(void)h;
	*out = L;
	return 0;
}

extern "C" void bhip_destroy(void *handle) {
	Handle *h = (Handle *)handle;
	if (!h) return;
	(void)hipSetDevice(h->device);
	if (h->stream) (void)hipStreamSynchronize(h->stream);
	if (h->sweep_stream) (void)hipStreamSynchronize(h->sweep_stream);
	if (h->pf_stream) (void)hipStreamSynchronize(h->pf_stream);
	if (h->post_stream) (void)hipStreamSynchronize(h->post_stream);
	if (h->stage_stream) (void)hipStreamSynchronize(h->stage_stream);
	for (StageSlot &S : h->slots) S.release_all();
	bhip_cov_release(h);
	bhip_paths_release(h);
	bhip_mates_release(h);
	if (h->hsc_pinned) (void)hipHostFree(h->hsc_pinned);
	if (h->nsel_pinned) (void)hipHostFree(h->nsel_pinned);
	for (Lane *L : h->lanes) lane_destroy(L);
	DBuf *all[] = {&h->ref_lane, &h->ref_off, &h->clump_len, &h->lut, &h->acx_lines, &h->acx_rec, &h->bad,
		&h->best, &h->out, &h->shared_ctr, &h->mins, &h->pairs, &h->sort_keys, &h->sort_keys2, &h->sort_idx,
		&h->sort_tmp, &h->out_sorted, &h->out_sorted2, &h->sort_scratch, &h->ref_order, &h->best_key};
	for (int o = 0; o < 2; ++o) {
		if (h->copy_pending[o] && h->ev_copied[o]) (void)hipEventSynchronize(h->ev_copied[o]);
		if (h->reg_ptr[o]) (void)hipHostUnregister(h->reg_ptr[o]);
		if (h->ev_copied[o]) (void)hipEventDestroy(h->ev_copied[o]);
	}
	if (h->ev_sorted) (void)hipEventDestroy(h->ev_sorted);
	if (h->copy_stream) (void)hipStreamDestroy(h->copy_stream);
	for (DBuf *b : all) b->release();
	for (auto &e : h->ev) if (e) (void)hipEventDestroy(e);
	if (h->stream) (void)hipStreamDestroy(h->stream);
	if (h->pf_stream) (void)hipStreamDestroy(h->pf_stream);
	if (h->stage_stream) (void)hipStreamDestroy(h->stage_stream);
	delete h;
}


extern "C" int bhip_init(int device, const void *edx_packed, const uint32_t *clump_len, uint32_t n_clumps, uint32_t tot_refs,
                         const uint32_t *acx_lens, const void *acx_lists, int acx_fmt, int K,
                         const uint32_t *badlist, uint32_t n_bad, const uint8_t score_lut[256], int xalpha, void **handle) {
	if (!handle) return fail(BHIP_E_ARG, "handle is NULL");
	*handle = nullptr;
	if (xalpha) return fail(BHIP_E_ARG, "xalpha (-x) databases are not supported on the device");
	if (!edx_packed || !clump_len || !n_clumps || !score_lut) return fail(BHIP_E_ARG, "empty database");
	if (acx_lens && (K < 4 || K > 15 || !acx_lists || (acx_fmt != 0 && acx_fmt != 1)))
		return fail(BHIP_E_ARG, "bad accelerator arguments (K=%d fmt=%d)", K, acx_fmt);
	if (!acx_lens && K && (K < 4 || K > 15)) return fail(BHIP_E_ARG, "bad accelerator word length K=%d", K);
	int ndev = 0;
	HIPCHK(hipGetDeviceCount(&ndev));
	if (device < 0 || device >= ndev) return fail(BHIP_E_DEVICE, "device %d not present (%d visible)", device, ndev);
	HIPCHK(hipSetDevice(device));
	Handle *h = new Handle();
	memset(h->ev, 0, sizeof h->ev);
	memset(&h->stats, 0, sizeof h->stats);
	h->device = device;
	hipDeviceProp_t prop;
	if (hipGetDeviceProperties(&prop, device) == hipSuccess) {
		h->n_cu = prop.multiProcessorCount; h->hbm = prop.totalGlobalMem;
		snprintf(h->dev_name, sizeof h->dev_name, "%s (%s)", prop.name, prop.gcnArchName);
	}
	if (h->n_cu <= 0) h->n_cu = 256;
	#define INITCHK(x) do { hipError_t e_ = (x); if (e_ != hipSuccess) { \
		fail(BHIP_E_DEVICE, "%s:%d %s: %s", __FILE__, __LINE__, #x, hipGetErrorString(e_)); bhip_destroy(h); return BHIP_E_DEVICE; } } while (0)
	#define INITRC(x) do { int rc_ = (x); if (rc_) { bhip_destroy(h); return rc_; } } while (0)
	INITCHK(hipStreamCreateWithFlags(&h->stream, hipStreamNonBlocking));
	h->sweep_stream = h->stream; h->post_stream = h->stream;
	INITCHK(hipStreamCreateWithFlags(&h->pf_stream, hipStreamNonBlocking));
	INITCHK(hipStreamCreateWithFlags(&h->stage_stream, hipStreamNonBlocking));
	for (auto &e : h->ev) INITCHK(hipEventCreate(&e));
	h->n_clumps = n_clumps; h->tot_refs = tot_refs;
	h->h_clump_len.assign(clump_len, clump_len + n_clumps);
	for (int a = 0; a < 16; ++a) {
		uint16_t m = 0;
		for (int b = 0; b < 16; ++b) if (score_lut[16 * a + b] == 0) m |= (uint16_t)(1u << b);
		h->mm.m[a] = m;
		uint8_t n = 0, bases = 0;
		for (int b = 1; b <= 4; ++b) if (m & (1u << b)) { bases |= (uint8_t)((b - 1) << (2 * n)); ++n; }
		h->alt.n[a] = n; h->alt.base[a] = bases;
	}
	std::vector<uint64_t> src_off(n_clumps + 1), dst_off(n_clumps + 1);
	src_off[0] = dst_off[0] = 0;
	for (uint32_t c = 0; c < n_clumps; ++c) {
		src_off[c + 1] = src_off[c] + clump_len[c] / 2u + (clump_len[c] & 1);
		dst_off[c + 1] = dst_off[c] + (clump_len[c] + 31) / 32u;
		if (clump_len[c] > h->max_clump_len) h->max_clump_len = clump_len[c];
	}
	{
		DBuf d_src, d_srcoff;
		INITRC(d_src.reserve(src_off[n_clumps] * 16 + 16));
		INITRC(d_srcoff.reserve((n_clumps + 1) * sizeof(uint64_t)));
		INITRC(h->ref_lane.reserve_exact(dst_off[n_clumps] * 256 + 256));
		INITRC(h->ref_off.reserve((n_clumps + 1) * sizeof(uint64_t)));
		INITRC(h->clump_len.reserve(n_clumps * sizeof(uint32_t)));
		INITRC(h->lut.reserve(256));
		INITCHK(hipMemcpyAsync(d_src.p, edx_packed, src_off[n_clumps] * 16, hipMemcpyHostToDevice, h->stream));
		INITCHK(hipMemcpyAsync(d_srcoff.p, src_off.data(), (n_clumps + 1) * sizeof(uint64_t), hipMemcpyHostToDevice, h->stream));
		INITCHK(hipMemcpyAsync(h->ref_off.p, dst_off.data(), (n_clumps + 1) * sizeof(uint64_t), hipMemcpyHostToDevice, h->stream));
		INITCHK(hipMemcpyAsync(h->clump_len.p, clump_len, n_clumps * sizeof(uint32_t), hipMemcpyHostToDevice, h->stream));
		INITCHK(hipMemcpyAsync(h->lut.p, score_lut, 256, hipMemcpyHostToDevice, h->stream));
		const uint32_t grid = std::min<uint32_t>(n_clumps, (uint32_t)h->n_cu * 8);
		hipLaunchKernelGGL(k_transpose_refs, dim3(grid), dim3(256), 0, h->stream, d_src.as<uint8_t>(), d_srcoff.as<uint64_t>(),
			h->clump_len.as<uint32_t>(), h->ref_off.as<uint64_t>(), n_clumps, h->ref_lane.as<uint4>());
		INITCHK(hipGetLastError());
		DBuf d_flag;
		INITRC(d_flag.reserve(sizeof(uint32_t)));
		INITCHK(hipMemsetAsync(d_flag.p, 0, sizeof(uint32_t), h->stream));
		hipLaunchKernelGGL(k_ref_symbol_scan, dim3((uint32_t)h->n_cu * 8), dim3(256), 0, h->stream, d_src.as<uint32_t>(), src_off[n_clumps] * 4, d_flag.as<uint32_t>());
		INITCHK(hipGetLastError());
		uint32_t any_other = 1;
		INITCHK(hipMemcpyAsync(&any_other, d_flag.p, sizeof(uint32_t), hipMemcpyDeviceToHost, h->stream));
		INITCHK(hipStreamSynchronize(h->stream));
		h->peq_rows = any_other ? 16u : 5u;
		d_src.release(); d_srcoff.release(); d_flag.release();
	}
	if (getenv("BHIP_DEBUG")) { size_t f_ = 0, t_ = 0; if (hipMemGetInfo(&f_, &t_) == hipSuccess) fprintf(stderr, "[bhip] references on the device (%.2f GB, upload buffer released): %.2f GB of the device's %.2f free\n", h->ref_lane.cap / 1e9, f_ / 1e9, t_ / 1e9); }
	h->acx_z = score_lut[16 * 5 + 5] != 0;
	if (acx_lens) INITRC(bhip_load_accelerator(h, acx_lens, acx_lists, acx_fmt, K, badlist, n_bad));
	else if (K) INITRC(bhip_build_accelerator(h, K, h->acx_z));
	INITRC(ensure_lanes(h, 1));
	if (const char *ev = getenv("BHIP_OPTS")) {
		std::string all(ev);
		for (size_t a = 0; a < all.size();) {
			size_t b = all.find(',', a); if (b == std::string::npos) b = all.size();
			const std::string kv = all.substr(a, b - a); a = b + 1;
			const size_t eq = kv.find('=');
			char *end = nullptr;
			const long long v = eq == std::string::npos ? 0 : strtoll(kv.c_str() + eq + 1, &end, 0);
			if (eq == std::string::npos || eq == 0 || !end || end == kv.c_str() + eq + 1 || *end) { fprintf(stderr, "[bhip] BHIP_OPTS: '%s' is not name=<integer>: ignored\n", kv.c_str()); continue; }
			if (bhip_set_option(h, kv.substr(0, eq).c_str(), v)) fprintf(stderr, "[bhip] BHIP_OPTS: %s: ignored\n", bhip_last_error());
		}
	}
	*handle = h;
	return BHIP_OK;
}


extern "C" int bhip_device_info(void *handle, char *name, int name_cap, int *n_cu, uint64_t *hbm_bytes) {
	Handle *h = (Handle *)handle;
	if (!h) return fail(BHIP_E_ARG, "null handle");
	if (name && name_cap > 0) snprintf(name, (size_t)name_cap, "%s", h->dev_name);
	if (n_cu) *n_cu = h->n_cu;
	if (hbm_bytes) *hbm_bytes = h->hbm;
	return BHIP_OK;
}

extern "C" int bhip_set_option(void *handle, const char *name, long long value) {
	Handle *h = (Handle *)handle;
	if (!h || !name) return fail(BHIP_E_ARG, "null argument");
	if (!strcmp(name, "prefilter_stride")) {
		if (value < 0 || value > 64) return fail(BHIP_E_ARG, "prefilter_stride must be 0 (auto) .. 64");
		h->opt_prefilter_stride = (int)value; return BHIP_OK;
	}
	if (!strcmp(name, "two_stage")) { h->opt_two_stage = value != 0; return BHIP_OK; }
	if (!strcmp(name, "host_routing")) { h->opt_host_routing = value != 0; return BHIP_OK; }
	if (!strcmp(name, "discard_staged")) { for (StageSlot &S : h->slots) if (S.state == 1) S.state = 0; h->res_valid = false; return BHIP_OK; }
	if (!strcmp(name, "lane_masks")) { h->opt_lane_masks = value != 0; return BHIP_OK; }
	if (!strcmp(name, "sweep_blocks")) { if (value < 1 || value > 8) return fail(BHIP_E_ARG, "sweep_blocks must be 1 .. 8"); h->opt_sweep_blocks = (int)value; return BHIP_OK; }
	if (!strcmp(name, "lane_min_entries")) { if (value < 1) return fail(BHIP_E_ARG, "lane_min_entries must be >= 1"); h->opt_lane_min = (int)value; return BHIP_OK; }
	if (!strcmp(name, "async_d2h")) { h->opt_async_d2h = value != 0; return BHIP_OK; }
	if (!strcmp(name, "seed_ahead")) { h->opt_seed_ahead = value != 0; return BHIP_OK; }
	if (!strcmp(name, "peq_ahead_blocks")) { if (value < 1 || value > 16) return fail(BHIP_E_ARG, "peq_ahead_blocks must be 1 .. 16"); h->opt_peq_ahead_blocks = (int)value; return BHIP_OK; }
	if (!strcmp(name, "seed_ahead_blocks")) { if (value < 0 || value > 64) return fail(BHIP_E_ARG, "seed_ahead_blocks must be 0 .. 64"); h->opt_seed_ahead_blocks = (int)value; return BHIP_OK; }
	if (!strcmp(name, "band_blocks")) { if (value < 0 || value > 1024) return fail(BHIP_E_ARG, "band_blocks must be 0 .. 1024"); h->opt_band_blocks = (int)value; return BHIP_OK; }
	if (!strcmp(name, "oversub")) { if (value < 1 || value > 16) return fail(BHIP_E_ARG, "oversub must be 1 .. 16"); h->opt_oversub = (int)value; return BHIP_OK; }
	if (!strcmp(name, "band")) { h->opt_no_band = value == 0; return BHIP_OK; }
	if (!strcmp(name, "prune")) { h->opt_prune = value != 0; return BHIP_OK; }
	if (!strcmp(name, "rescore_reg")) { h->opt_rescore_reg = value != 0; return BHIP_OK; }
	if (!strcmp(name, "seed_min_need")) { if (value < -1 || value > 255) return fail(BHIP_E_ARG, "seed_min_need must be -1 (by rule) or 0 .. 255"); h->opt_seed_min_need = (int)value; return BHIP_OK; }
	if (!strcmp(name, "seed_drop_len")) { if (value < 0 || value > (1 << 24)) return fail(BHIP_E_ARG, "seed_drop_len must be 0 .. 2^24"); h->opt_seed_drop_len = (int)value; return BHIP_OK; }
	if (!strcmp(name, "prefilter_waves")) { if (value < 0 || value > 16) return fail(BHIP_E_ARG, "prefilter_waves must be 0 .. 16"); h->opt_pf_waves = (int)value; return BHIP_OK; }
	if (!strcmp(name, "prefilter_algo")) { if (value < -1 || value > 1) return fail(BHIP_E_ARG, "prefilter_algo must be -1, 0 or 1"); h->opt_pf_algo = (int)value; return BHIP_OK; }
	if (!strcmp(name, "prefilter_table")) { if (value != 0 && (value < 9 || value > 11)) return fail(BHIP_E_ARG, "prefilter_table must be 0, 9, 10 or 11"); h->opt_pf_table = (int)value; return BHIP_OK; }
	if (!strcmp(name, "prefilter_cw")) { if (value < 0 || value > 2) return fail(BHIP_E_ARG, "prefilter_cw must be 0, 1 or 2"); h->opt_pf_cw = (int)value; return BHIP_OK; }
	if (!strcmp(name, "prefilter_bytes")) { h->opt_pf_bytes = value != 0; return BHIP_OK; }
	if (!strcmp(name, "prefilter_rb")) { if (value != 0 && (value < 2 || value > 4)) return fail(BHIP_E_ARG, "prefilter_rb must be 0, 2, 3 or 4"); h->opt_pf_rb = (int)value; return BHIP_OK; }
	if (!strcmp(name, "cov_event_cap")) { if (value < 0) return fail(BHIP_E_ARG, "cov_event_cap must be >= 0 bytes (0 = a fifth of the free memory)"); h->opt_cov_event_cap = value; return BHIP_OK; }
	if (!strcmp(name, "lanes")) {
		if (value < 1 || value > BHIP_MAX_LANES) return fail(BHIP_E_ARG, "lanes must be 1 .. %d", BHIP_MAX_LANES);
		h->opt_lanes = (int)value; for (StageSlot &S : h->slots) { S.state = 0; S.st_valid = false; } return BHIP_OK;
	}
	return fail(BHIP_E_ARG, "unknown option '%s'", name);
}

extern "C" int bhip_get_stats(void *handle, BhipStats *out) {
	Handle *h = (Handle *)handle;
	if (!h || !out) return fail(BHIP_E_ARG, "null argument");
	*out = h->stats;
	return BHIP_OK;
}

int ensure_lanes(Handle *h, uint32_t n) {
	while (h->lanes.size() < n) { Lane *L = nullptr; int rc = lane_create(h, &L); if (rc) return rc; h->lanes.push_back(L); }
	return 0;
}
```

burst_amd/csrc/bhip_kernels.hip:

```cpp
#include <hip/hip_runtime.h>
#include <stdint.h>
#include <type_traits>
#include "burst_hip.h"
#include "bhip_internal.h"

__global__ void k_transpose_refs(const uint8_t *__restrict__ src, const uint64_t *__restrict__ src_off,
                                 const uint32_t *__restrict__ clump_len, const uint64_t *__restrict__ dst_off,
                                 uint32_t n_clumps, uint4 *__restrict__ dst_lane) {
	const uint32_t z = threadIdx.x & 15, g = threadIdx.x >> 4, gpb = blockDim.x >> 4;
	for (uint32_t c = blockIdx.x; c < n_clumps; c += gridDim.x) {
		const uint32_t L = clump_len[c], nrows = (L + 1) >> 1, nchunks = (L + 31) >> 5;
		const uint8_t *s = src + src_off[c] * 16;
		for (uint32_t t = g; t < nchunks; t += gpb) {
			uint32_t w[4] = {0, 0, 0, 0};
			#pragma unroll
			for (int i = 0; i < 16; ++i) {
				uint32_t row = 16 * t + i;
				uint32_t b = row < nrows ? s[(uint64_t)row * 16 + z] : 0u;
				w[i >> 2] |= b << (8 * (i & 3));
			}
			dst_lane[dst_off[c] * 16 + (uint64_t)z * nchunks + t] = make_uint4(w[0], w[1], w[2], w[3]);
		}
	}
}


__global__ __launch_bounds__(256) void k_build_peq(const uint8_t *__restrict__ qcodes, const uint64_t *__restrict__ qoff,
                            const uint32_t *__restrict__ qlist, uint32_t n_list, int NW, int prefix_len,
                            BhipMatchMask mm, uint32_t *__restrict__ peq, const uint32_t *__restrict__ qpack, uint32_t qw, uint32_t n_rows) {
	__shared__ uint32_t s_mm[16];
	__shared__ uint32_t s_out[256 * 16 + 256];
	const uint32_t tid = threadIdx.x;
	if (tid < 16) s_mm[tid] = mm.m[tid];
	const uint32_t QB = 256u / (uint32_t)NW, per_q = 16u * (uint32_t)NW;
	const uint32_t lq = tid / (uint32_t)NW, w = tid % (uint32_t)NW;
	for (uint32_t q0 = blockIdx.x * QB; q0 < n_list; q0 += gridDim.x * QB) {
		__syncthreads();
		const uint32_t li = q0 + lq;
		if (lq < QB && li < n_list) {
			const uint32_t q = qlist ? qlist[li] : li;
			const uint64_t b = qoff[q];
			int len = (int)(qoff[q + 1] - b);
			if (prefix_len > 0 && len > prefix_len) len = prefix_len;
			const int shift = 32 * NW - len;
			uint32_t row[16];
			if (qpack) {
				const int pb = 32 * (int)w - shift, j0 = pb >> 3;
				const uint32_t *qp = qpack + (uint64_t)q * qw;
				uint32_t D[5], dd[4];
				#pragma unroll
				for (int i = 0; i < 5; ++i) D[i] = (j0 + i >= 0 && (uint32_t)(j0 + i) < qw) ? qp[j0 + i] : 0u;
				#pragma unroll
				for (int i = 0; i < 4; ++i) dd[i] = __builtin_amdgcn_alignbit(D[i + 1], D[i], 4u * ((uint32_t)pb & 7u));
				#pragma unroll
				for (int j = 0; j < 16; ++j) {
					const uint32_t lo = pb + j < 0 ? 0xFFFFu : s_mm[(dd[j >> 3] >> (4 * (j & 7))) & 15u];
					const uint32_t hi = pb + j + 16 < 0 ? 0xFFFFu : s_mm[(dd[2 + (j >> 3)] >> (4 * (j & 7))) & 15u];
					row[j] = lo | (hi << 16);
				}
			} else {
				#pragma unroll
				for (int j = 0; j < 16; ++j) {
					const int p0 = 32 * (int)w + j - shift, p1 = p0 + 16;
					const uint32_t lo = p0 < 0 ? 0xFFFFu : s_mm[qcodes[b + p0] & 15], hi = p1 < 0 ? 0xFFFFu : s_mm[qcodes[b + p1] & 15];
					row[j] = lo | (hi << 16);
				}
			}
			#pragma unroll
			for (int st = 0; st < 4; ++st) {
				const int j = 8 >> st;
				const uint32_t msk = st == 0 ? 0x00FF00FFu : st == 1 ? 0x0F0F0F0Fu : st == 2 ? 0x33333333u : 0x55555555u;
				#pragma unroll
				for (int k = 0; k < 16; ++k) if (!(k & j)) {
					const uint32_t t = ((row[k] >> j) ^ row[k + j]) & msk;
					row[k + j] ^= t;
					row[k] ^= t << j;
				}
			}
			#pragma unroll
			for (int c = 0; c < 16; ++c) s_out[lq * (per_q + 1) + (uint32_t)c * (uint32_t)NW + w] = row[c];
		}
		__syncthreads();
		const uint32_t nq = n_list - q0 < QB ? n_list - q0 : QB;
		const uint32_t per_w = n_rows * (uint32_t)NW, total = nq * per_w;
		uint32_t *dst = peq + (uint64_t)q0 * per_q;
		const uint32_t st_q = 256u / per_w, st_r = 256u % per_w;
		uint32_t oq = tid / per_w, orr = tid % per_w;
		for (uint32_t idx = tid; idx < total; idx += 256) {
			dst[oq * per_q + orr] = s_out[oq * (per_q + 1) + orr];
			oq += st_q; orr += st_r;
			if (orr >= per_w) { orr -= per_w; ++oq; }
		}
	}
}

template <int NW>
__device__ __forceinline__ void myers_step(const uint32_t (&Eq)[NW], uint32_t (&Pv)[NW], uint32_t (&Mv)[NW], int &score) {
	uint32_t Ph[NW], Mh[NW];
	uint32_t carry = 0;
	#pragma unroll
	for (int w = 0; w < NW; ++w) {
		uint32_t co;
		const uint32_t s = __builtin_addc(Eq[w] & Pv[w], Pv[w], carry, &co);
		carry = co;
		const uint32_t Xh = (s ^ Pv[w]) | Eq[w];
		Ph[w] = Mv[w] | ~(Xh | Pv[w]);
		Mh[w] = Pv[w] & Xh;
	}
	uint32_t cP = 0, cM = 0;
	#pragma unroll
	for (int w = 0; w < NW; ++w) {
		uint32_t co;
		Ph[w] = __builtin_addc(Ph[w], Ph[w], cP, &co); cP = co;
		Mh[w] = __builtin_addc(Mh[w], Mh[w], cM, &co); cM = co;
	}
	score += (int)cP - (int)cM;
	#pragma unroll
	for (int w = 0; w < NW; ++w) {
		const uint32_t Xv = Eq[w] | Mv[w];
		Pv[w] = Mh[w] | ~(Xv | Ph[w]);
		Mv[w] = Ph[w] & Xv;
	}
}

template <int NW>
__global__ __launch_bounds__(256) void k_myers(
		const uint2 *__restrict__ pairs, const uint32_t *__restrict__ n_pairs_dev, uint64_t n_pairs_host,
		uint32_t n_clumps_implicit,
		uint32_t li_base,
		const uint32_t *__restrict__ qlist,
		const uint32_t *__restrict__ peq, const uint64_t *__restrict__ qoff, const uint16_t *__restrict__ qemac,
		const uint32_t *__restrict__ qsix,
		const uint4 *__restrict__ ref, const uint64_t *__restrict__ ref_off, const uint32_t *__restrict__ clump_len,
		uint32_t tot_refs,
		BhipRawHit *__restrict__ raw, uint32_t *__restrict__ n_raw, uint32_t raw_cap, uint32_t *__restrict__ best,
		uint8_t *__restrict__ mins_out, unsigned long long *__restrict__ col_sum, unsigned long long *__restrict__ qlen_sum) {
	__shared__ __attribute__((aligned(16))) uint32_t s_peq[16][16 * NW];
	const uint32_t tid = threadIdx.x, g = tid >> 4, z = tid & 15, rot = 4 * (g & 3);
	const uint64_t n_pairs = n_pairs_dev ? ((uint64_t)*n_pairs_dev < n_pairs_host ? (uint64_t)*n_pairs_dev : n_pairs_host) : n_pairs_host;
	const uint64_t n_tiles = (n_pairs + 15) >> 4;
	unsigned long long my_cols = 0, my_qlen = 0;
	for (uint64_t tile = blockIdx.x; tile < n_tiles; tile += gridDim.x) {
		const uint64_t p = tile * 16 + g;
		const bool live = p < n_pairs;
		uint32_t li = 0, c = 0;
		if (live) {
			if (pairs) { const uint2 pr = pairs[p]; li = pr.x; c = pr.y; }
			else { li = li_base + (uint32_t)(p / n_clumps_implicit); c = (uint32_t)(p % n_clumps_implicit); }
		}
		__syncthreads();
		if (live) {
			const uint32_t *src = peq + ((uint64_t)li * 16 + z) * NW;
			uint32_t *dstrow = &s_peq[g][((z + rot) & 15) * NW];
			#pragma unroll
			for (int w = 0; w < NW; ++w) dstrow[w] = src[w];
		}
		__syncthreads();
		if (!live) continue;
		const uint32_t q = qlist ? qlist[li] : li;
		const uint32_t m = (uint32_t)(qoff[q + 1] - qoff[q]), E = qemac[q];
		const uint32_t L = clump_len[c], nchunks = (L + 31) >> 5;
		uint32_t Pv[NW], Mv[NW];
		#pragma unroll
		for (int w = 0; w < NW; ++w) {
			const int lo = 32 * NW - (int)m - 32 * w;
			Pv[w] = lo <= 0 ? 0xFFFFFFFFu : (lo >= 32 ? 0u : (0xFFFFFFFFu << lo));
			Mv[w] = 0;
		}
		int score = (int)m, bestS = 0x7FFFFFFF;
		uint32_t first = 0, last = 0;
		const uint4 *rp = ref + ref_off[c] * 16 + (uint64_t)z * nchunks;
		const uint32_t *tab = &s_peq[g][0];
		for (uint32_t t = 0; t < nchunks; ++t) {
			const uint4 ch = rp[t];
			const uint32_t dw[4] = {ch.x, ch.y, ch.z, ch.w};
			#pragma unroll
			for (int i = 0; i < 32; ++i) {
				const uint32_t sym = (dw[i >> 3] >> (4 * (i & 7))) & 15u;
				const uint32_t *row = tab + ((sym + rot) & 15u) * NW;
				uint32_t Eq[NW];
				#pragma unroll
				for (int w = 0; w < NW; ++w) Eq[w] = row[w];
				myers_step<NW>(Eq, Pv, Mv, score);
				const uint32_t col = t * 32 + i + 1;
				const bool lt = score < bestS, le = score <= bestS;
				bestS = lt ? score : bestS;
				first = lt ? col : first;
				last = le ? col : last;
			}
		}
		const uint32_t refIx = c * 16 + z;
		const bool hit = (uint32_t)bestS <= E && refIx < tot_refs;
		if (mins_out) mins_out[p * 16 + z] = (uint32_t)bestS <= E ? (uint8_t)bestS : (uint8_t)255;
		if (hit && raw) {
			const uint32_t pos = atomicAdd(n_raw, 1u);
			if (pos < raw_cap) {
				BhipRawHit h; h.q = q; h.refIx = refIx; h.ed = (uint32_t)bestS; h.e_first = first; h.e_last = last;
				h.m = m; h.L = L; h.six = qsix ? qsix[q] : q; h.rbase = ref_off[c] * 16 + (uint64_t)z * nchunks;
				raw[pos] = h;
			}
			if (best) atomicMin(&best[qsix ? qsix[q] : q], (uint32_t)bestS);
		}
		if (z == 0) { my_cols += L; my_qlen += m; }
	}
	if (col_sum && my_cols) { atomicAdd(col_sum, my_cols); atomicAdd(qlen_sum, my_qlen); }
}

__global__ __launch_bounds__(64) void k_myers_long(
		const uint2 *__restrict__ pairs, const uint32_t *__restrict__ n_pairs_dev, uint64_t n_pairs_host, uint32_t n_clumps_implicit, uint32_t li_base,
		const uint32_t *__restrict__ qlist, const uint32_t *__restrict__ peq, const uint64_t *__restrict__ qoff, const uint16_t *__restrict__ qemac,
		const uint32_t *__restrict__ qsix, const uint4 *__restrict__ ref, const uint64_t *__restrict__ ref_off, const uint32_t *__restrict__ clump_len,
		uint32_t tot_refs, BhipRawHit *__restrict__ raw, uint32_t *__restrict__ n_raw, uint32_t raw_cap, uint32_t *__restrict__ best,
		uint8_t *__restrict__ mins_out, unsigned long long *__restrict__ col_sum, unsigned long long *__restrict__ qlen_sum, uint32_t NW) {
	extern __shared__ uint32_t s_long[];
	const uint32_t tid = threadIdx.x, g = tid >> 4, z = tid & 15;
	uint32_t *sP = s_long + tid, *sM = s_long + (size_t)NW * 64 + tid;
	const uint64_t n_pairs = n_pairs_dev ? ((uint64_t)*n_pairs_dev < n_pairs_host ? (uint64_t)*n_pairs_dev : n_pairs_host) : n_pairs_host;
	const uint64_t n_tiles = (n_pairs + 3) >> 2;
	unsigned long long my_cols = 0, my_qlen = 0;
	for (uint64_t tile = blockIdx.x; tile < n_tiles; tile += gridDim.x) {
		const uint64_t p = tile * 4 + g;
		if (p >= n_pairs) continue;
		uint32_t li, c;
		if (pairs) { const uint2 pr = pairs[p]; li = pr.x; c = pr.y; }
		else { li = li_base + (uint32_t)(p / n_clumps_implicit); c = (uint32_t)(p % n_clumps_implicit); }
		const uint32_t q = qlist ? qlist[li] : li;
		const uint32_t m = (uint32_t)(qoff[q + 1] - qoff[q]), E = qemac[q];
		const uint32_t L = clump_len[c], nchunks = (L + 31) >> 5;
		for (uint32_t w = 0; w < NW; ++w) {
			const int lo = 32 * (int)NW - (int)m - 32 * (int)w;
			sP[w * 64] = lo <= 0 ? 0xFFFFFFFFu : (lo >= 32 ? 0u : (0xFFFFFFFFu << lo));
			sM[w * 64] = 0;
		}
		int score = (int)m, bestS = 0x7FFFFFFF;
		uint32_t first = 0, last = 0;
		const uint4 *rp = ref + ref_off[c] * 16 + (uint64_t)z * nchunks;
		const uint32_t *tab = peq + (uint64_t)li * 16 * NW;
		for (uint32_t t = 0; t < nchunks; ++t) {
			const uint4 ch = rp[t];
			#pragma unroll 1
			for (uint32_t i = 0; i < 32; ++i) {
				const uint32_t d = i < 8 ? ch.x : i < 16 ? ch.y : i < 24 ? ch.z : ch.w;
				const uint32_t *row = tab + ((d >> (4 * (i & 7))) & 15u) * NW;
				uint32_t carry = 0, cP = 0, cM = 0;
				for (uint32_t w = 0; w < NW; ++w) {
					const uint32_t Eq = row[w], Pv = sP[w * 64], Mv = sM[w * 64];
					uint32_t co;
					const uint32_t s = __builtin_addc(Eq & Pv, Pv, carry, &co); carry = co;
					const uint32_t Xh = (s ^ Pv) | Eq;
					uint32_t Ph = Mv | ~(Xh | Pv), Mh = Pv & Xh;
					Ph = __builtin_addc(Ph, Ph, cP, &co); cP = co;
					Mh = __builtin_addc(Mh, Mh, cM, &co); cM = co;
					const uint32_t Xv = Eq | Mv;
					sP[w * 64] = Mh | ~(Xv | Ph);
					sM[w * 64] = Ph & Xv;
				}
				score += (int)cP - (int)cM;
				const uint32_t col = t * 32 + i + 1;
				const bool lt = score < bestS, le = score <= bestS;
				bestS = lt ? score : bestS;
				first = lt ? col : first;
				last = le ? col : last;
			}
		}
		const uint32_t refIx = c * 16 + z;
		const bool hit = (uint32_t)bestS <= E && refIx < tot_refs;
		if (mins_out) mins_out[p * 16 + z] = (uint32_t)bestS <= E ? (uint8_t)bestS : (uint8_t)255;
		if (hit && raw) {
			const uint32_t pos = atomicAdd(n_raw, 1u);
			if (pos < raw_cap) {
				BhipRawHit h; h.q = q; h.refIx = refIx; h.ed = (uint32_t)bestS; h.e_first = first; h.e_last = last;
				h.m = m; h.L = L; h.six = qsix ? qsix[q] : q; h.rbase = ref_off[c] * 16 + (uint64_t)z * nchunks;
				raw[pos] = h;
			}
			if (best) atomicMin(&best[qsix ? qsix[q] : q], (uint32_t)bestS);
		}
		if (z == 0) { my_cols += L; my_qlen += m; }
	}
	if (col_sum && my_cols) { atomicAdd(col_sum, my_cols); atomicAdd(qlen_sum, my_qlen); }
}

template <int NWP>
__global__ __launch_bounds__(256) void k_myers_prefix(
		const uint2 *__restrict__ pairs, const uint32_t *__restrict__ n_pairs_dev, uint64_t n_pairs_host,
		uint32_t n_clumps_implicit, uint32_t li_base,
		const uint32_t *__restrict__ qlist, const uint32_t *__restrict__ peqp, const uint64_t *__restrict__ qoff,
		const uint16_t *__restrict__ qemac,
		const uint4 *__restrict__ ref, const uint64_t *__restrict__ ref_off, const uint32_t *__restrict__ clump_len,
		uint32_t tot_refs, BhipWin *__restrict__ wins, uint32_t *__restrict__ n_wins, uint32_t win_cap,
		unsigned long long *__restrict__ col_sum, unsigned long long *__restrict__ qlen_sum, uint32_t *__restrict__ cls_seen,
		const uint32_t *__restrict__ qsix) {
	__shared__ __attribute__((aligned(16))) uint32_t s_peq[16][16 * NWP];
	const uint32_t tid = threadIdx.x, g = tid >> 4, z = tid & 15;
	const uint64_t n_pairs = n_pairs_dev ? ((uint64_t)*n_pairs_dev < n_pairs_host ? (uint64_t)*n_pairs_dev : n_pairs_host) : n_pairs_host;
	const uint64_t n_tiles = (n_pairs + 15) >> 4;
	unsigned long long my_cols = 0, my_qlen = 0;
	for (uint64_t tile = blockIdx.x; tile < n_tiles; tile += gridDim.x) {
		const uint64_t p = tile * 16 + g;
		const bool live = p < n_pairs;
		uint32_t li = 0, c = 0;
		if (live) {
			if (pairs) { const uint2 pr = pairs[p]; li = pr.x; c = pr.y; }
			else { li = li_base + (uint32_t)(p / n_clumps_implicit); c = (uint32_t)(p % n_clumps_implicit); }
		}
		__syncthreads();
		if (live) {
			const uint32_t *src = peqp + ((uint64_t)li * 16 + z) * NWP;
// ... 559 lines not shown
		else if (len <= 1024u) for (uint32_t p = 0; p < npos; p += st) W += (vb[p >> 5] >> (p & 31u)) & 1u;
		else for (uint32_t p = 0; p < npos; p += st) {
			uint32_t ok = 1u;
			for (uint32_t k = 0; k < K; ++k) ok &= (sym(p + k) - 1u) < 4u ? 1u : 0u;
			W += ok;
		}
		return (int)W - (int)(E * ((K + st - 1) / st));
	};
	const uint32_t smin = (len - K) / 254 + 1, smax = K > smin ? K : smin;
	uint32_t best_s = 0; int best_n = 0;
	if (stride_opt > 0) { best_s = (uint32_t)stride_opt > smin ? (uint32_t)stride_opt : smin; best_n = need_of(best_s); }
	else {
		for (uint32_t st = smax; st >= smin; --st) { const int n = need_of(st); if (n >= 3) { best_s = st; best_n = n; break; } if (st == smin) break; }
		if (!best_s) for (uint32_t st = smin; st <= smax; ++st) { const int n = need_of(st); if (n > best_n) { best_n = n; best_s = st; } }
		if (!best_s) { best_s = smin; best_n = need_of(smin); }
	}
	if (best_n < 1) best_n = 0;
	if (best_n > 0xFFFF) best_n = 0xFFFF;
	const bool ex = !clean && best_s == K && best_n > 0 && xk > 0;
	return (best_s & 255u) | ((uint32_t)best_n << 8) | (ex ? xk << 24 | usedk << 28 : 0u);
}

__global__ __launch_bounds__(256) void k_route(
		const uint64_t *__restrict__ qoff, const uint32_t *__restrict__ qpack, uint32_t qw, const uint16_t *__restrict__ qemac,
		const uint32_t *__restrict__ qsix, const uint8_t *__restrict__ qflags, uint32_t n_q, uint32_t n_shared, uint32_t n_lanes,
		int has_acx, int K, int stride_opt,
		uint32_t *__restrict__ plan, uint8_t *__restrict__ key_out, uint32_t *__restrict__ idx_out, BhipStageInfo *__restrict__ info, BhipAlt alt) {
	__shared__ uint32_t s_count[256], s_maxE[BHIP_ROUTE_KEYS / 2], s_maxw[BHIP_ROUTE_KEYS / 2], s_seed[BHIP_ROUTE_KEYS / 2], s_maxlen[16], s_nent[16], s_misc[4];
	const uint32_t tid = threadIdx.x;
	s_count[tid] = 0;
	if (tid < BHIP_ROUTE_KEYS / 2) { s_maxE[tid] = 0; s_maxw[tid] = 0; s_seed[tid] = 0; }
	if (tid < 16) { s_maxlen[tid] = 0; s_nent[tid] = 0; }
	if (tid < 4) s_misc[tid] = 0;
	__syncthreads();
	for (uint32_t i = blockIdx.x * 256 + tid; i < n_q; i += gridDim.x * 256) {
		const uint64_t b = qoff[i];
		const uint64_t len64 = qoff[i + 1] - b;
		uint32_t key = BHIP_ROUTE_SKIP, pl = 1u;
		if (len64 > BHIP_MAX_QLEN || len64 > 8ull * qw) { if (!atomicExch(&info->err, 1u)) { info->err_i = i; info->err_len = (uint32_t)(len64 > 0xFFFFFFFFull ? 0xFFFFFFFFull : len64); } }
		else if (qsix && qsix[i] >= n_shared) { if (!atomicExch(&info->err, 2u)) info->err_i = i; }
		else if (len64) {
			const uint32_t len = (uint32_t)len64, E = qemac[i];
			const uint32_t *qp = qpack + (uint64_t)i * qw;
			uint32_t n_zero = 0, n_other = 0;
			for (uint32_t j = 0; j < (len + 7) >> 3; ++j) {
				const uint32_t d = qp[j], nsym = len - 8 * j < 8 ? len - 8 * j : 8u;
				const uint32_t valid = nsym >= 8 ? 0x88888888u : (0x88888888u & ((1u << (4 * nsym)) - 1u));
				const uint32_t zero = ~(((d & 0x77777777u) + 0x77777777u) | d);
				const uint32_t ge5 = d | ((d << 1) & ((d << 2) | (d << 3)));
				n_zero += __popc(zero & valid);
				n_other += __popc((zero | ge5) & valid);
			}
			if (n_zero) atomicOr(&s_misc[0], 1u);
			const uint32_t six = qsix ? qsix[i] : i;
			const uint32_t l = (uint32_t)(((unsigned long long)six * n_lanes) / n_shared);
			const uint32_t cls = len <= 64 ? 0u : len <= 128 ? 1u : len <= 192 ? 2u : len <= 256 ? 3u : len <= 320 ? 4u : len <= 512 ? 5u : len <= 1024 ? 6u : 7u;
			uint32_t ex = qflags ? (qflags[i] == BHIP_Q_EXHAUSTIVE) : !has_acx;
			if (!has_acx) ex = 1;
			if (!ex) {
				uint32_t vb[32];
				const bool clean = n_other == 0;
				if (!clean && len >= (uint32_t)K && len <= 1024u) {
					for (uint32_t w = 0; w < 32; ++w) vb[w] = 0;
					uint32_t run = 0;
					for (uint32_t p = 0; p < len; ++p) {
						const uint32_t c = (qp[p >> 3] >> (4 * (p & 7u))) & 15u;
						run = (c - 1u) < 4u ? run + 1 : 0;
						if (p + 1 >= (uint32_t)K && run >= (uint32_t)K) { const uint32_t w0 = p + 1 - K; vb[w0 >> 5] |= 1u << (w0 & 31u); }
					}
				}
				pl = bhip_seed_plan(len, E, (uint32_t)K, stride_opt, clean, vb, qp, alt);
				if (BHIP_PLAN_NEED(pl) == 0) ex = 1;
			}
			const uint32_t lc = l * BHIP_N_CLASSES + cls;
			key = lc * 2 + ex;
			atomicAdd(&s_count[key], 1u);
			atomicMax(&s_maxE[lc], E);
			if (!ex && len >= (uint32_t)K) {
				const uint32_t nwd = (len - K) / (pl & 255u) + 1 + BHIP_PLAN_USED(pl);
				atomicMax(&s_maxw[lc], nwd);
				atomicAdd(&s_seed[lc], nwd);
			}
			atomicMax(&s_maxlen[l], len);
			atomicAdd(&s_nent[l], 1u);
			atomicMax(&s_misc[1], E);
		}
		plan[i] = pl;
		key_out[i] = (uint8_t)key;
		idx_out[i] = i;
	}
	__syncthreads();
	if (s_count[tid]) atomicAdd(&info->count[tid], s_count[tid]);
	if (tid < BHIP_ROUTE_KEYS / 2) {
		if (s_maxE[tid]) atomicMax(&info->maxE[tid], s_maxE[tid]);
		if (s_maxw[tid]) atomicMax(&info->maxwords[tid], s_maxw[tid]);
		if (s_seed[tid]) atomicAdd(&info->seed_words[tid], (unsigned long long)s_seed[tid]);
	}
	if (tid < 16) { if (s_maxlen[tid]) { atomicMax(&info->maxlen_lane[tid], s_maxlen[tid]); atomicMax(&info->maxlen_all, s_maxlen[tid]); } if (s_nent[tid]) atomicAdd(&info->n_entries_lane[tid], s_nent[tid]); }
	if (tid == 0) { if (s_misc[0]) atomicOr(&info->junk, 1u); if (s_misc[1]) atomicMax(&info->maxE_all, s_misc[1]); }
}

template <bool WIDE>
__global__ __launch_bounds__(64) void k_rescore(
		const BhipRawHit *__restrict__ raw, const uint32_t *__restrict__ n_raw_dev, uint32_t raw_cap,
		const uint32_t *__restrict__ wide_in, const uint32_t *__restrict__ n_wide_in,
		const uint32_t *__restrict__ best, int all_hits,
		const uint8_t *__restrict__ qcodes, const uint64_t *__restrict__ qoff,
		const uint32_t *__restrict__ qsix, const uint8_t *__restrict__ qrc,
		const uint8_t *__restrict__ refb, const uint64_t *__restrict__ ref_off, const uint32_t *__restrict__ clump_len,
		const uint8_t *__restrict__ lut,
		BhipHit *__restrict__ out, uint32_t *__restrict__ n_out, uint32_t out_cap,
		uint32_t *__restrict__ wide_out, uint32_t *__restrict__ n_wide_out,
		uint32_t *__restrict__ g_scratch, unsigned long long *__restrict__ scratch_used, unsigned long long scratch_cap,
		uint32_t *__restrict__ err_flags,
		const uint32_t *__restrict__ qpack, uint32_t band_rows, uint32_t qw, uint32_t rw) {
	extern __shared__ __attribute__((aligned(16))) uint32_t smem[];
	__shared__ uint32_t s_mm[16];
	const uint32_t tid = threadIdx.x;
	uint32_t *s_band = smem + tid;
	uint32_t *s_q = smem + (size_t)(band_rows + 1) * 64 + tid;
	uint32_t *s_r = s_q + (size_t)qw * 64;
	if (tid < 16) { uint32_t m = 0; for (int r = 0; r < 16; ++r) m |= (lut[16 * tid + r] == 0 ? 1u : 0u) << r | (lut[16 * tid + r] != 255 ? 1u : 0u) << (16 + r); s_mm[tid] = m; }
	__syncthreads();
	const uint32_t *refw = (const uint32_t *)refb;
	uint32_t n = wide_in ? *n_wide_in : *n_raw_dev;
	if (n > raw_cap) n = raw_cap;
	for (uint32_t ii = blockIdx.x * 64 + tid; ii < n; ii += gridDim.x * 64) {
		const uint32_t i = wide_in ? wide_in[ii] : ii;
		const BhipRawHit h = raw[i];
		const uint32_t q = h.q, six = qsix ? qsix[q] : q;
		if (!all_hits && h.ed != best[six]) continue;
		const uint32_t B = h.ed, c = h.refIx >> 4, z = h.refIx & 15, L = clump_len[c], nchunks = (L + 31) >> 5;
		const uint64_t qb = qoff[q];
		const int m = (int)(qoff[q + 1] - qb);
		const int e2 = (int)(h.e_last < L ? h.e_last : L);
		if (B == 0) {
			const uint32_t pos = atomicAdd(n_out, 1u);
			if (pos < out_cap) {
				BhipHit o; o.q = q; o.refIx = h.refIx; o.finalPos = (uint32_t)e2; o.score = 1.0f - 0.0f / (float)m;
				o.ed = 0; o.gapR = 0; o.gapQ = 0; o.rc = qrc ? qrc[q] : 0;
				out[pos] = o;
				bhip_hit_rank(n_out, pos, q);
			}
			continue;
		}
		const int e1 = (int)h.e_first;
		const int dlo = e1 - m - (int)B, dhi = e2 - m + (int)B, Wd = dhi - dlo + 1;
		uint32_t *band; uint32_t stride;
		if (!WIDE) {
			if (Wd > (int)band_rows) {
				const uint32_t pos = atomicAdd(n_wide_out, 1u);
				wide_out[pos] = i;
				continue;
			}
			band = s_band; stride = 64;
		} else {
			const unsigned long long off = atomicAdd(scratch_used, (unsigned long long)(Wd + 1));
			if (off + Wd + 1 > scratch_cap) { atomicOr(err_flags, 2u); continue; }
			band = g_scratch + off; stride = 1;
		}
		const uint64_t cbase = ref_off[c];
		if (B > 254u) { atomicOr(err_flags, 1u); continue; }
		constexpr uint32_t SS = 18, GS = 10;
		const uint32_t INVALID = (512u << SS) | (255u << GS);
		const uint32_t STEP_U = (1u << SS) + 1u + (1u << 8), STEP_L = (1u << SS) - (1u << GS) + (2u << 8);
		const int j8_0 = (dlo - 1) >> 3, j8_1 = (dlo + m + Wd) >> 3;
		const bool pre = qpack && (uint32_t)m <= 8 * qw && (uint32_t)(j8_1 - j8_0 + 1) <= rw;
		if (pre) {
			const uint32_t *qp = qpack + (uint64_t)q * qw;
			for (uint32_t j = 0; j < (uint32_t)(m + 7) >> 3; ++j) s_q[j * 64] = qp[j];
			for (int j = j8_0; j <= j8_1; ++j) s_r[(uint32_t)(j - j8_0) * 64] = ref_dword_lane(refw, cbase, z, j, nchunks);
		}
		auto rdw = [&](int j8) -> uint32_t { return pre ? s_r[(uint32_t)(j8 - j8_0) * 64] : ref_dword_lane(refw, cbase, z, j8, nchunks); };
		for (int k = 0; k <= Wd; ++k) {
			const int x = dlo + k;
			band[(uint32_t)k * stride] = (k < Wd && x >= 0 && x <= (int)L) ? (255u << GS) : INVALID;
		}
		uint32_t qdw = 0;
		for (int y = 1; y <= m; ++y) {
			uint32_t qc;
			if (pre) { if (((y - 1) & 7) == 0) qdw = s_q[(uint32_t)((y - 1) >> 3) * 64]; qc = (qdw >> (4 * ((y - 1) & 7))) & 15u; }
			else qc = qcodes[qb + y - 1] & 15u;
			const uint32_t mrow = s_mm[qc], m1 = mrow >> 16;
			const uint32_t col0 = (uint32_t)y <= B ? (((uint32_t)y << SS) | (255u << GS) | (uint32_t)y) : INVALID;
			const int x0 = y + dlo;
			uint32_t left = (x0 - 1 == 0) ? col0 : INVALID;
			int pos = x0 - 1;
			uint32_t dw = rdw(pos >> 3);
			uint32_t prev_sym = (y == 1) ? ((rdw((pos - 1) >> 3) >> (4 * ((pos - 1) & 7))) & 15u) : 0u;
			uint32_t dg = band[0];
			for (int k = 0; k < Wd; ++k, ++pos) {
				const int x = x0 + k;
				if ((pos & 7) == 0 && k) dw = rdw(pos >> 3);
				const uint32_t r = (dw >> (4 * (pos & 7))) & 15u;
				const uint32_t up = band[(uint32_t)(k + 1) * stride];
				uint32_t cell;
				if (x < 1) cell = (x == 0) ? col0 : INVALID;
				else if (x > (int)L) cell = INVALID;
				else {
					const uint32_t cst = ((mrow >> r) & 1u) ? 0u : (((m1 >> r) & 1u) ? 1u : 255u);
					if (y == 1) {
						uint32_t hh = 0;
						if (cst == 1 && x >= 2) hh = (mrow >> prev_sym) & 1u;
						cell = cst == 255u ? INVALID : ((cst << SS) | ((255u - hh) << GS));
					} else {
						const uint32_t cD = dg + (cst << SS), cU = up + STEP_U, cL = left + STEP_L;
						uint32_t cm = cD < cU ? cD : cU;
						cm = cm < cL ? cm : cL;
						cm &= ~0x300u;
						cell = (cm >> SS) > B ? INVALID : cm;
					}
				}
				prev_sym = r;
				band[(uint32_t)k * stride] = cell;
				left = cell;
				dg = up;
			}
		}
		uint32_t bkey = 0xFFFFFFFFu, bv = 0, fin = 0xFFFFFFFFu;
		for (int k = 0; k < Wd; ++k) {
			const int x = m + dlo + k;
			if (x < 1 || x > (int)L) continue;
			const uint32_t cell = band[(uint32_t)k * stride], key = cell >> GS;
			if (key < bkey) { bkey = key; bv = cell & 255u; }
		}
		for (int k = 0; k < Wd; ++k) {
			const int x = m + dlo + k;
			if (x < 1 || x > (int)L) continue;
			if ((band[(uint32_t)k * stride] >> GS) == bkey) fin = (uint32_t)x;
		}
		const uint32_t bs = bkey >> 8, bh = 255u - (bkey & 255u);
		if (bs != B) { atomicOr(err_flags, 1u); continue; }
		const uint32_t pos = atomicAdd(n_out, 1u);
		if (pos < out_cap) {
			BhipHit o;
			o.q = q; o.refIx = h.refIx; o.finalPos = fin;
			o.score = 1.0f - (float)bs / ((float)m + (float)bh);
			o.ed = (uint8_t)B; o.gapR = (uint8_t)bv; o.gapQ = (uint8_t)bh; o.rc = qrc ? qrc[q] : 0;
			out[pos] = o;
			bhip_hit_rank(n_out, pos, q);
		}
	}
}

__global__ __launch_bounds__(256) void k_rescore_classify(
		const BhipRawHit *__restrict__ raw, const uint32_t *__restrict__ n_raw_dev, uint32_t raw_cap,
		const uint32_t *__restrict__ best, int all_hits, const uint64_t *__restrict__ qoff,
		const uint32_t *__restrict__ qsix, const uint8_t *__restrict__ qrc, const uint32_t *__restrict__ clump_len,
		BhipHit *__restrict__ out, uint32_t *__restrict__ n_out, uint32_t out_cap,
		uint32_t *__restrict__ lists, uint32_t *__restrict__ counts, uint32_t *__restrict__ wide, uint32_t *__restrict__ n_wide,
		uint32_t band_rows, int use_reg) {
	__shared__ uint32_t s_cnt[12], s_base[12];
	uint32_t n = *n_raw_dev;
	if (n > raw_cap) n = raw_cap;
	const uint32_t tid = threadIdx.x;
	for (uint32_t chunk = blockIdx.x * 1024u; chunk < n; chunk += gridDim.x * 1024u) {
		if (tid < 12) s_cnt[tid] = 0;
		__syncthreads();
		int bucket[4]; uint32_t rank[4], e2v[4], mv[4], qv[4], rv[4];
		#pragma unroll
		for (int t = 0; t < 4; ++t) {
			const uint32_t i = chunk + (uint32_t)t * 256u + tid;
			bucket[t] = -1; rank[t] = 0; e2v[t] = 0; mv[t] = 0; qv[t] = 0; rv[t] = 0;
			if (i < n) {
				const BhipRawHit h = raw[i];
				if (all_hits || h.ed == best[h.six]) {
					const uint32_t L = h.L;
					const uint32_t e2 = h.e_last < L ? h.e_last : L;
					qv[t] = h.q; rv[t] = h.refIx; e2v[t] = e2;
					if (h.ed == 0) { bucket[t] = 11; mv[t] = h.m; }
					else {
						const uint32_t Wd = e2 - h.e_first + 2 * h.ed + 1;
						int bk = !use_reg || h.ed > 254u ? 9 : Wd <= 4 ? 0 : Wd <= 6 ? 1 : Wd <= 8 ? 2 : Wd <= 12 ? 3 : Wd <= 16 ? 4 : Wd <= 24 ? 5 : Wd <= 32 ? 6 : Wd <= 40 ? 7 : Wd <= 48 ? 8 : 9;
						if (Wd > band_rows && bk == 9) bk = 10;
						bucket[t] = bk;
					}
					rank[t] = atomicAdd(&s_cnt[bucket[t]], 1u);
				}
			}
		}
		__syncthreads();
		if (tid < 12 && s_cnt[tid]) s_base[tid] = atomicAdd(tid == 11 ? n_out : tid == 10 ? n_wide : &counts[tid], s_cnt[tid]);
		__syncthreads();
		#pragma unroll
		for (int t = 0; t < 4; ++t) {
			const uint32_t i = chunk + (uint32_t)t * 256u + tid;
			const int bk = bucket[t];
			if (bk < 0) continue;
			const uint32_t pos = s_base[bk] + rank[t];
			if (bk == 11) {
				if (pos < out_cap) {
					BhipHit o; o.q = qv[t]; o.refIx = rv[t]; o.finalPos = e2v[t]; o.score = 1.0f - 0.0f / (float)mv[t];
					o.ed = 0; o.gapR = 0; o.gapQ = 0; o.rc = qrc ? qrc[qv[t]] : 0;
					out[pos] = o;
					bhip_hit_rank(n_out, pos, qv[t]);
				}
			} else if (bk == 10) wide[pos] = i;
			else lists[(size_t)bk * raw_cap + pos] = i;
		}
		__syncthreads();
	}
}

template <int WB>
__device__ __forceinline__ void rescore_reg_one(
		const BhipRawHit *__restrict__ hp, bool live, uint32_t *s_mm, uint32_t fastq, uint32_t lane,
		const uint64_t *__restrict__ qoff, const uint8_t *__restrict__ qrc, const uint32_t *__restrict__ qpack, uint32_t qw,
		const uint32_t *__restrict__ refw, const uint64_t *__restrict__ ref_off, const uint32_t *__restrict__ clump_len,
		BhipHit *__restrict__ out, uint32_t *__restrict__ n_out, uint32_t out_cap, uint32_t *__restrict__ err_flags) {
	constexpr int NW = (WB + 7) / 8 + 1;
	constexpr uint32_t SS = 18, GS = 10;
	const uint32_t INVALID = (512u << SS) | (255u << GS), Z0 = 255u << GS;
	const uint32_t STEP_U = (1u << SS) + 1u + (1u << 8), STEP_L = (1u << SS) - (1u << GS) + (2u << 8);
	uint32_t bkey = 0xFFFFFFFFu, bv = 0, fin = 0xFFFFFFFFu, m = 0, B = 0, hq = 0, hrefIx = 0;
	if (live) {
		const uint32_t q = hp->q;
		hq = q; hrefIx = hp->refIx;
		B = hp->ed;
		const uint32_t h_first = hp->e_first, h_last = hp->e_last;
		const uint32_t L = hp->L, nchunks = (L + 31) >> 5;
		m = hp->m;
		const int e2 = (int)(h_last < L ? h_last : L), e1 = (int)h_first;
		const int dlo = e1 - (int)m - (int)B, Wd = e2 - e1 + 2 * (int)B + 1;
		const uint64_t rbase = hp->rbase;
		const uint32_t LIM = (B + 1) << SS;
		uint32_t bd[WB + 1];
		#pragma unroll
		for (int k = 0; k < WB; ++k) { const int x = dlo + k; bd[k] = (k < Wd && x >= 0 && x <= (int)L) ? Z0 : INVALID; }
		bd[WB] = INVALID;
		int p = dlo, j8 = dlo >> 3;
		uint32_t d[NW];
		#pragma unroll
		for (int i = 0; i < NW; ++i) d[i] = ref_dword_at(refw, rbase, j8 + i, nchunks);
		auto all_acgt = [&]() { uint32_t bad = 0;
			#pragma unroll
			for (int i = 0; i < NW; ++i) bad |= (d[i] - 0x11111111u) & 0xCCCCCCCCu;
			return bad == 0; };
		bool dclean = all_acgt();
		int jn = j8 + NW;
		uint4 ahead = ref_chunk_at(refw, rbase, jn >> 2, nchunks);
		const uint32_t *qp = qpack + (uint64_t)q * qw;
		uint32_t qd = qp[0], q_next = qw > 1 ? qp[1] : 0u;
		uint32_t prev_sym = (ref_dword_at(refw, rbase, (p - 1) >> 3, nchunks) >> (4 * ((p - 1) & 7))) & 15u;
		for (int y = 1; y <= (int)m; ++y) {
			const uint32_t qi = (uint32_t)(y - 1);
			if ((qi & 7u) == 0 && qi) { qd = q_next; q_next = (qi >> 3) + 1 < qw ? qp[(qi >> 3) + 1] : 0u; }
			const uint32_t qc = (qd >> (4 * (qi & 7u))) & 15u;
			const uint32_t col0 = (uint32_t)y <= B ? (((uint32_t)y << SS) | Z0 | (uint32_t)y) : INVALID;
			const int x0 = y + dlo;
			const bool fast_row = y > 1 && x0 >= 1 && dclean && ((fastq >> qc) & 1u);
			const uint32_t mrow = fast_row ? 0u : s_mm[qc];
			const uint32_t m1 = mrow >> 16;
			uint32_t dd[NW - 1];
			{
				const uint32_t sh = 4u * ((uint32_t)p & 7u);
				#pragma unroll
				for (int i = 0; i < NW - 1; ++i) dd[i] = __builtin_amdgcn_alignbit(d[i + 1], d[i], sh);
			}
			const int kmax = (Wd - 1) < ((int)L - x0) ? (Wd - 1) : ((int)L - x0);
			if (y == 1) {
				#pragma unroll
				for (int k = 0; k < WB; ++k) {
					const int x = x0 + k;
					const uint32_t r = (dd[k >> 3] >> (4 * (k & 7))) & 15u;
					const uint32_t cst = ((mrow >> r) & 1u) ? 0u : (((m1 >> r) & 1u) ? 1u : 255u);
					uint32_t hh = 0;
					if (cst == 1 && x >= 2) hh = (mrow >> prev_sym) & 1u;
					uint32_t cell = cst == 255u ? INVALID : ((cst << SS) | ((255u - hh) << GS));
					if (x < 1) cell = x == 0 ? col0 : INVALID;
					if (k > kmax) cell = INVALID;
					prev_sym = r;
					bd[k] = cell;
				}
			} else if (fast_row) {
				uint32_t nz[NW - 1];
				#pragma unroll
				for (int i = 0; i < NW - 1; ++i) { const uint32_t x = dd[i] ^ (qc * 0x11111111u); nz[i] = ((x & 0x77777777u) + 0x77777777u) | x; }
				uint32_t left = (x0 - 1 == 0) ? col0 : INVALID;
				uint32_t dg = bd[0];
				#pragma unroll
				for (int k = 0; k < WB; ++k) {
					const uint32_t up = bd[k + 1];
					const uint32_t cD = dg + (((nz[k >> 3] >> (4 * (k & 7) + 3)) & 1u) << SS), cU = up + STEP_U, cL = left + STEP_L;
					uint32_t cm = cD < cU ? cD : cU;
					cm = cm < cL ? cm : cL;
					cm &= ~0x300u;
					uint32_t cell = cm >= LIM ? INVALID : cm;
					if (k > kmax) cell = INVALID;
					bd[k] = cell;
					left = cell;
					dg = up;
				}
			} else {
				uint32_t left = (x0 - 1 == 0) ? col0 : INVALID;
				uint32_t dg = bd[0];
				#pragma unroll
				for (int k = 0; k < WB; ++k) {
					const uint32_t r = (dd[k >> 3] >> (4 * (k & 7))) & 15u;
					const uint32_t up = bd[k + 1];
					const uint32_t cstS = ((mrow >> r) & 1u) ? 0u : (((m1 >> r) & 1u) ? (1u << SS) : (255u << SS));
					const uint32_t cD = dg + cstS, cU = up + STEP_U, cL = left + STEP_L;
					uint32_t cm = cD < cU ? cD : cU;
					cm = cm < cL ? cm : cL;
					cm &= ~0x300u;
					uint32_t cell = cm >= LIM ? INVALID : cm;
					if (x0 < 1) { const int x = x0 + k; if (x < 1) cell = x == 0 ? col0 : INVALID; }
					if (k > kmax) cell = INVALID;
					bd[k] = cell;
					left = cell;
					dg = up;
				}
			}
			++p;
			if ((p & 7) == 0) {
				#pragma unroll
				for (int i = 0; i < NW - 1; ++i) d[i] = d[i + 1];
				d[NW - 1] = pick4(ahead, (uint32_t)jn & 3u);
				dclean = all_acgt();
				++j8; ++jn;
				if ((jn & 3) == 0) ahead = ref_chunk_at(refw, rbase, jn >> 2, nchunks);
			}
		}
		#pragma unroll
		for (int k = 0; k < WB; ++k) {
			const int x = (int)m + dlo + k;
			if (k < Wd && x >= 1 && x <= (int)L) { const uint32_t key = bd[k] >> GS; if (key < bkey) { bkey = key; bv = bd[k] & 255u; } }
		}
		#pragma unroll
		for (int k = 0; k < WB; ++k) {
			const int x = (int)m + dlo + k;
			if (k < Wd && x >= 1 && x <= (int)L && (bd[k] >> GS) == bkey) fin = (uint32_t)x;
		}
	}
	const uint32_t bs = bkey >> 8, bh = 255u - (bkey & 255u);
	const bool ok = live && bs == B;
	if (live && !ok) atomicOr(err_flags, 1u);
	const unsigned long long bm = __ballot(ok);
	if (bm) {
		uint32_t base = 0;
		if (lane == (uint32_t)__builtin_ctzll(bm)) base = atomicAdd(n_out, (uint32_t)__popcll(bm));
		base = __shfl(base, __builtin_ctzll(bm));
		if (ok) {
			const uint32_t pos = base + __popcll(bm & ((1ull << lane) - 1ull));
			if (pos < out_cap) {
				BhipHit o;
				o.q = hq; o.refIx = hrefIx; o.finalPos = fin;
				o.score = 1.0f - (float)bs / ((float)m + (float)bh);
				o.ed = (uint8_t)B; o.gapR = (uint8_t)bv; o.gapQ = (uint8_t)bh; o.rc = qrc ? qrc[hq] : 0;
				out[pos] = o;
				bhip_hit_rank(n_out, pos, hq);
			}
		}
	}
}

template <int SET>
__global__ __launch_bounds__(64) void k_rescore_reg(
		const BhipRawHit *__restrict__ raw, const uint32_t *__restrict__ lists, const uint32_t *__restrict__ counts, uint32_t raw_cap,
		const uint64_t *__restrict__ qoff, const uint8_t *__restrict__ qrc, const uint32_t *__restrict__ qpack, uint32_t qw,
		const uint8_t *__restrict__ refb, const uint64_t *__restrict__ ref_off, const uint32_t *__restrict__ clump_len,
		const uint8_t *__restrict__ lut,
		BhipHit *__restrict__ out, uint32_t *__restrict__ n_out, uint32_t out_cap, uint32_t *__restrict__ err_flags) {
	__shared__ uint32_t s_mm[16];
	const uint32_t tid = threadIdx.x;
	if (tid < 16) { uint32_t mm = 0; for (int r = 0; r < 16; ++r) mm |= (lut[16 * tid + r] == 0 ? 1u : 0u) << r | (lut[16 * tid + r] != 255 ? 1u : 0u) << (16 + r); s_mm[tid] = mm; }
	__syncthreads();
	uint32_t fastq = 0;
	for (uint32_t qc = 1; qc <= 4; ++qc) if ((s_mm[qc] & 0x1Eu) == (1u << qc)) fastq |= 1u << qc;
	const uint32_t *refw = (const uint32_t *)refb;
#define BHIP_RS_RUN(b, WB) { \
		uint32_t n = counts[b]; if (n > raw_cap) n = raw_cap; \
		const uint32_t *lst = lists + (size_t)(b) * raw_cap; \
		const uint32_t n_round = (n + 63u) & ~63u; \
		for (uint32_t i = blockIdx.x * 64 + tid; i < n_round; i += gridDim.x * 64) { \
			const bool live = i < n; \
			rescore_reg_one<WB>(raw + (live ? lst[i] : 0u), live, s_mm, fastq, tid, qoff, qrc, qpack, qw, refw, ref_off, clump_len, out, n_out, out_cap, err_flags); \
		} }
	if (SET == 0) { BHIP_RS_RUN(0, 4) BHIP_RS_RUN(1, 6) BHIP_RS_RUN(2, 8) }
	else if (SET == 3) { BHIP_RS_RUN(3, 12) }
	else if (SET == 1) { BHIP_RS_RUN(4, 16) BHIP_RS_RUN(5, 24) }
	else { BHIP_RS_RUN(6, 32) BHIP_RS_RUN(7, 40) BHIP_RS_RUN(8, 48) }
#undef BHIP_RS_RUN
}
template __global__ void k_rescore_reg<0>(const BhipRawHit *, const uint32_t *, const uint32_t *, uint32_t, const uint64_t *, const uint8_t *, const uint32_t *, uint32_t,
	const uint8_t *, const uint64_t *, const uint32_t *, const uint8_t *, BhipHit *, uint32_t *, uint32_t, uint32_t *);
template __global__ void k_rescore_reg<1>(const BhipRawHit *, const uint32_t *, const uint32_t *, uint32_t, const uint64_t *, const uint8_t *, const uint32_t *, uint32_t,
	const uint8_t *, const uint64_t *, const uint32_t *, const uint8_t *, BhipHit *, uint32_t *, uint32_t, uint32_t *);
template __global__ void k_rescore_reg<2>(const BhipRawHit *, const uint32_t *, const uint32_t *, uint32_t, const uint64_t *, const uint8_t *, const uint32_t *, uint32_t,
	const uint8_t *, const uint64_t *, const uint32_t *, const uint8_t *, BhipHit *, uint32_t *, uint32_t, uint32_t *);
template __global__ void k_rescore_reg<3>(const BhipRawHit *, const uint32_t *, const uint32_t *, uint32_t, const uint64_t *, const uint8_t *, const uint32_t *, uint32_t,
	const uint8_t *, const uint64_t *, const uint32_t *, const uint8_t *, BhipHit *, uint32_t *, uint32_t, uint32_t *);

template __global__ void k_rescore<false>(const BhipRawHit *, const uint32_t *, uint32_t, const uint32_t *, const uint32_t *, const uint32_t *, int,
	const uint8_t *, const uint64_t *, const uint32_t *, const uint8_t *, const uint8_t *, const uint64_t *, const uint32_t *, const uint8_t *,
	BhipHit *, uint32_t *, uint32_t, uint32_t *, uint32_t *, uint32_t *, unsigned long long *, unsigned long long, uint32_t *,
	const uint32_t *, uint32_t, uint32_t, uint32_t);
template __global__ void k_rescore<true>(const BhipRawHit *, const uint32_t *, uint32_t, const uint32_t *, const uint32_t *, const uint32_t *, int,
	const uint8_t *, const uint64_t *, const uint32_t *, const uint8_t *, const uint8_t *, const uint64_t *, const uint32_t *, const uint8_t *,
	BhipHit *, uint32_t *, uint32_t, uint32_t *, uint32_t *, uint32_t *, unsigned long long *, unsigned long long, uint32_t *,
	const uint32_t *, uint32_t, uint32_t, uint32_t);
```

Measured before the change: 617.9 million.

## Process eight interior rows per step in register rescore band kernel

Moves the banded rescore DP into a shared header and adds a path that handles eight query rows at once when the reference and query dwords are clean ACGT and the row lies in the band interior. It skips per-row boundary checks and symbol extraction in that path. It also precomputes the match masks and fastq flags on the host, and adds an early exit for blocks that have no work in their set. The cost is more code and register pressure for small band widths, plus a new correctness risk in the interior-row bounds logic.

```diff
diff --git a/burst_amd/csrc/bhip_align.hip b/burst_amd/csrc/bhip_align.hip
--- a/burst_amd/csrc/bhip_align.hip
+++ b/burst_amd/csrc/bhip_align.hip
@@ -651,8 +651,8 @@
 			constexpr int SET = decltype(set)::value;
 			const uint32_t grid = (uint32_t)h->n_cu * std::min<uint32_t>(32u, blocks_per_cu((const void *)k_rescore_reg<SET>, 64, 0)) * (uint32_t)h->opt_oversub;
 			hipLaunchKernelGGL(k_rescore_reg<SET>, dim3(grid), dim3(64), 0, po, L->raw.as<BhipRawHit>(), L->rs_lists.as<uint32_t>(), dc->n_rs, (uint32_t)L->raw_cap,
-				h->cur->qoff.as<uint64_t>(), rc_or_null(h), h->cur->qpack.as<uint32_t>(), qw_g,
-				R.bytes(), R.off, R.len, h->lut.as<uint8_t>(), h->out.as<BhipHit>(), &sc->n_out, (uint32_t)h->out_cap, &sc->err);
+				rc_or_null(h), h->cur->qpack.as<uint32_t>(), qw_g,
+				R.bytes(), h->rs_mm.as<uint32_t>(), h->opt_rescore_rows8, h->out.as<BhipHit>(), &sc->n_out, (uint32_t)h->out_cap, &sc->err);
 		});
 		HIPCHK(hipGetLastError());
 	}
diff --git a/burst_amd/csrc/bhip_handle.h b/burst_amd/csrc/bhip_handle.h
--- a/burst_amd/csrc/bhip_handle.h
+++ b/burst_amd/csrc/bhip_handle.h
@@ -70,8 +70,8 @@
 	uint32_t *, uint8_t *, uint32_t *, BhipStageInfo *, BhipAlt);
 __global__ void k_rescore_classify(const BhipRawHit *, const uint32_t *, uint32_t, const uint32_t *, int, const uint64_t *, const uint32_t *, const uint8_t *,
 	const uint32_t *, BhipHit *, uint32_t *, uint32_t, uint32_t *, uint32_t *, uint32_t *, uint32_t *, uint32_t, int);
-template <int SET> __global__ void k_rescore_reg(const BhipRawHit *, const uint32_t *, const uint32_t *, uint32_t, const uint64_t *, const uint8_t *, const uint32_t *, uint32_t,
-	const uint8_t *, const uint64_t *, const uint32_t *, const uint8_t *, BhipHit *, uint32_t *, uint32_t, uint32_t *);
+template <int SET> __global__ void k_rescore_reg(const BhipRawHit *, const uint32_t *, const uint32_t *, uint32_t, const uint8_t *, const uint32_t *, uint32_t,
+	const uint8_t *, const uint32_t *, int, BhipHit *, uint32_t *, uint32_t, uint32_t *);
 int bhip_fail_msg(int code, const char *fmt, ...) __attribute__((format(printf, 2, 3)));
 #define fail(...) bhip_fail_msg(__VA_ARGS__)
 inline bool bhip_trace_sync() { static const bool on = getenv("BHIP_TRACE_SYNC") != nullptr; return on; }
@@ -307,6 +307,7 @@
 	hipStream_t post_stream = nullptr;
 	hipEvent_t ev[EV_COUNT];
 	uint32_t n_clumps = 0, tot_refs = 0, max_clump_len = 0;
+	DBuf rs_mm;
 	DBuf ref_lane, ref_off, clump_len, lut;
 	BhipMatchMask mm;
 	BhipAlt alt;
@@ -357,6 +358,7 @@
 	int opt_prune = 1;
 	int opt_lane_min = 32768;
 	int opt_rescore_reg = 1;
+	int opt_rescore_rows8 = 1;
 	int opt_pf_waves = 0;
 	int opt_pf_algo = -1;
 	int opt_pf_table = 0;
diff --git a/burst_amd/csrc/bhip_init.hip b/burst_amd/csrc/bhip_init.hip
--- a/burst_amd/csrc/bhip_init.hip
+++ b/burst_amd/csrc/bhip_init.hip
@@ -1,4 +1,5 @@
 #include "bhip_handle.h"
+#include "bhip_rescore_band.h"
 
 static thread_local char g_err[512] = "";
 
@@ -73,7 +74,7 @@
 	if (h->hsc_pinned) (void)hipHostFree(h->hsc_pinned);
 	if (h->nsel_pinned) (void)hipHostFree(h->nsel_pinned);
 	for (Lane *L : h->lanes) lane_destroy(L);
-	DBuf *all[] = {&h->ref_lane, &h->ref_off, &h->clump_len, &h->lut, &h->acx_lines, &h->acx_rec, &h->bad,
+	DBuf *all[] = {&h->ref_lane, &h->ref_off, &h->clump_len, &h->lut, &h->rs_mm, &h->acx_lines, &h->acx_rec, &h->bad,
 		&h->best, &h->out, &h->shared_ctr, &h->mins, &h->pairs, &h->sort_keys, &h->sort_keys2, &h->sort_idx,
 		&h->sort_tmp, &h->out_sorted, &h->out_sorted2, &h->sort_scratch, &h->ref_order, &h->best_key};
 	for (int o = 0; o < 2; ++o) {
@@ -149,11 +150,15 @@
 		INITRC(h->ref_off.reserve((n_clumps + 1) * sizeof(uint64_t)));
 		INITRC(h->clump_len.reserve(n_clumps * sizeof(uint32_t)));
 		INITRC(h->lut.reserve(256));
+		INITRC(h->rs_mm.reserve(BHIP_RS_MM_WORDS * sizeof(uint32_t)));
 		INITCHK(hipMemcpyAsync(d_src.p, edx_packed, src_off[n_clumps] * 16, hipMemcpyHostToDevice, h->stream));
 		INITCHK(hipMemcpyAsync(d_srcoff.p, src_off.data(), (n_clumps + 1) * sizeof(uint64_t), hipMemcpyHostToDevice, h->stream));
 		INITCHK(hipMemcpyAsync(h->ref_off.p, dst_off.data(), (n_clumps + 1) * sizeof(uint64_t), hipMemcpyHostToDevice, h->stream));
 		INITCHK(hipMemcpyAsync(h->clump_len.p, clump_len, n_clumps * sizeof(uint32_t), hipMemcpyHostToDevice, h->stream));
 		INITCHK(hipMemcpyAsync(h->lut.p, score_lut, 256, hipMemcpyHostToDevice, h->stream));
+		uint32_t rs_mm[BHIP_RS_MM_WORDS];
+		bhip_rescore_masks(score_lut, rs_mm);
+		INITCHK(hipMemcpyAsync(h->rs_mm.p, rs_mm, sizeof rs_mm, hipMemcpyHostToDevice, h->stream));
 		const uint32_t grid = std::min<uint32_t>(n_clumps, (uint32_t)h->n_cu * 8);
 		hipLaunchKernelGGL(k_transpose_refs, dim3(grid), dim3(256), 0, h->stream, d_src.as<uint8_t>(), d_srcoff.as<uint64_t>(),
 			h->clump_len.as<uint32_t>(), h->ref_off.as<uint64_t>(), n_clumps, h->ref_lane.as<uint4>());
@@ -222,6 +227,7 @@
 	if (!strcmp(name, "band")) { h->opt_no_band = value == 0; return BHIP_OK; }
 	if (!strcmp(name, "prune")) { h->opt_prune = value != 0; return BHIP_OK; }
 	if (!strcmp(name, "rescore_reg")) { h->opt_rescore_reg = value != 0; return BHIP_OK; }
+	if (!strcmp(name, "rescore_rows8")) { h->opt_rescore_rows8 = value != 0; return BHIP_OK; }
 	if (!strcmp(name, "seed_min_need")) { if (value < -1 || value > 255) return fail(BHIP_E_ARG, "seed_min_need must be -1 (by rule) or 0 .. 255"); h->opt_seed_min_need = (int)value; return BHIP_OK; }
 	if (!strcmp(name, "seed_drop_len")) { if (value < 0 || value > (1 << 24)) return fail(BHIP_E_ARG, "seed_drop_len must be 0 .. 2^24"); h->opt_seed_drop_len = (int)value; return BHIP_OK; }
 	if (!strcmp(name, "prefilter_waves")) { if (value < 0 || value > 16) return fail(BHIP_E_ARG, "prefilter_waves must be 0 .. 16"); h->opt_pf_waves = (int)value; return BHIP_OK; }
diff --git a/burst_amd/csrc/bhip_kernels.hip b/burst_amd/csrc/bhip_kernels.hip
--- a/burst_amd/csrc/bhip_kernels.hip
+++ b/burst_amd/csrc/bhip_kernels.hip
@@ -3,6 +3,7 @@
 #include <type_traits>
 #include "burst_hip.h"
 #include "bhip_internal.h"
+#include "bhip_rescore_band.h"
 
 __global__ void k_transpose_refs(const uint8_t *__restrict__ src, const uint64_t *__restrict__ src_off,
                                  const uint32_t *__restrict__ clump_len, const uint64_t *__restrict__ dst_off,
@@ -1168,135 +1169,33 @@
 	}
 }
 
+struct RefLaneAt {
+	const uint32_t *__restrict__ refw; uint64_t rbase; uint32_t nchunks;
+	__device__ __forceinline__ uint32_t dword(int j8) const { return ref_dword_at(refw, rbase, j8, nchunks); }
+	__device__ __forceinline__ uint4 chunk(int t4) const { return ref_chunk_at(refw, rbase, t4, nchunks); }
+	__device__ __forceinline__ uint4 chunk_clamped(int t4) const {
+		const bool in = t4 >= 0 && (uint32_t)t4 < nchunks;
+		const uint4 v = ((const uint4 *)refw)[rbase + (in ? (uint32_t)t4 : 0u)];
+		return in ? v : make_uint4(0, 0, 0, 0);
+	}
+};
+
 template <int WB>
 __device__ __forceinline__ void rescore_reg_one(
-		const BhipRawHit *__restrict__ hp, bool live, uint32_t *s_mm, uint32_t fastq, uint32_t lane,
-		const uint64_t *__restrict__ qoff, const uint8_t *__restrict__ qrc, const uint32_t *__restrict__ qpack, uint32_t qw,
-		const uint32_t *__restrict__ refw, const uint64_t *__restrict__ ref_off, const uint32_t *__restrict__ clump_len,
+		const BhipRawHit *__restrict__ hp, bool live, const uint32_t *s_mm, uint32_t fastq, bool rows8, uint32_t lane,
+		const uint8_t *__restrict__ qrc, const uint32_t *__restrict__ qpack, uint32_t qw,
+		const uint32_t *__restrict__ refw,
 		BhipHit *__restrict__ out, uint32_t *__restrict__ n_out, uint32_t out_cap, uint32_t *__restrict__ err_flags) {
-	constexpr int NW = (WB + 7) / 8 + 1;
-	constexpr uint32_t SS = 18, GS = 10;
-	const uint32_t INVALID = (512u << SS) | (255u << GS), Z0 = 255u << GS;
-	const uint32_t STEP_U = (1u << SS) + 1u + (1u << 8), STEP_L = (1u << SS) - (1u << GS) + (2u << 8);
 	uint32_t bkey = 0xFFFFFFFFu, bv = 0, fin = 0xFFFFFFFFu, m = 0, B = 0, hq = 0, hrefIx = 0;
 	if (live) {
 		const uint32_t q = hp->q;
 		hq = q; hrefIx = hp->refIx;
 		B = hp->ed;
-		const uint32_t h_first = hp->e_first, h_last = hp->e_last;
-		const uint32_t L = hp->L, nchunks = (L + 31) >> 5;
+		const uint32_t L = hp->L;
 		m = hp->m;
-		const int e2 = (int)(h_last < L ? h_last : L), e1 = (int)h_first;
-		const int dlo = e1 - (int)m - (int)B, Wd = e2 - e1 + 2 * (int)B + 1;
-		const uint64_t rbase = hp->rbase;
-		const uint32_t LIM = (B + 1) << SS;
-		uint32_t bd[WB + 1];
-		#pragma unroll
-		for (int k = 0; k < WB; ++k) { const int x = dlo + k; bd[k] = (k < Wd && x >= 0 && x <= (int)L) ? Z0 : INVALID; }
-		bd[WB] = INVALID;
-		int p = dlo, j8 = dlo >> 3;
-		uint32_t d[NW];
-		#pragma unroll
-		for (int i = 0; i < NW; ++i) d[i] = ref_dword_at(refw, rbase, j8 + i, nchunks);
-		auto all_acgt = [&]() { uint32_t bad = 0;
-			#pragma unroll
-			for (int i = 0; i < NW; ++i) bad |= (d[i] - 0x11111111u) & 0xCCCCCCCCu;
-			return bad == 0; };
-		bool dclean = all_acgt();
-		int jn = j8 + NW;
-		uint4 ahead = ref_chunk_at(refw, rbase, jn >> 2, nchunks);
-		const uint32_t *qp = qpack + (uint64_t)q * qw;
-		uint32_t qd = qp[0], q_next = qw > 1 ? qp[1] : 0u;
-		uint32_t prev_sym = (ref_dword_at(refw, rbase, (p - 1) >> 3, nchunks) >> (4 * ((p - 1) & 7))) & 15u;
-		for (int y = 1; y <= (int)m; ++y) {
-			const uint32_t qi = (uint32_t)(y - 1);
-			if ((qi & 7u) == 0 && qi) { qd = q_next; q_next = (qi >> 3) + 1 < qw ? qp[(qi >> 3) + 1] : 0u; }
-			const uint32_t qc = (qd >> (4 * (qi & 7u))) & 15u;
-			const uint32_t col0 = (uint32_t)y <= B ? (((uint32_t)y << SS) | Z0 | (uint32_t)y) : INVALID;
-			const int x0 = y + dlo;
-			const bool fast_row = y > 1 && x0 >= 1 && dclean && ((fastq >> qc) & 1u);
-			const uint32_t mrow = fast_row ? 0u : s_mm[qc];
-			const uint32_t m1 = mrow >> 16;
-			uint32_t dd[NW - 1];
-			{
-				const uint32_t sh = 4u * ((uint32_t)p & 7u);
-				#pragma unroll
-				for (int i = 0; i < NW - 1; ++i) dd[i] = __builtin_amdgcn_alignbit(d[i + 1], d[i], sh);
-			}
-			const int kmax = (Wd - 1) < ((int)L - x0) ? (Wd - 1) : ((int)L - x0);
-			if (y == 1) {
-				#pragma unroll
-				for (int k = 0; k < WB; ++k) {
-					const int x = x0 + k;
-					const uint32_t r = (dd[k >> 3] >> (4 * (k & 7))) & 15u;
-					const uint32_t cst = ((mrow >> r) & 1u) ? 0u : (((m1 >> r) & 1u) ? 1u : 255u);
-					uint32_t hh = 0;
-					if (cst == 1 && x >= 2) hh = (mrow >> prev_sym) & 1u;
-					uint32_t cell = cst == 255u ? INVALID : ((cst << SS) | ((255u - hh) << GS));
-					if (x < 1) cell = x == 0 ? col0 : INVALID;
-					if (k > kmax) cell = INVALID;
-					prev_sym = r;
-					bd[k] = cell;
-				}
-			} else if (fast_row) {
-				uint32_t nz[NW - 1];
-				#pragma unroll
-				for (int i = 0; i < NW - 1; ++i) { const uint32_t x = dd[i] ^ (qc * 0x11111111u); nz[i] = ((x & 0x77777777u) + 0x77777777u) | x; }
-				uint32_t left = (x0 - 1 == 0) ? col0 : INVALID;
-				uint32_t dg = bd[0];
-				#pragma unroll
-				for (int k = 0; k < WB; ++k) {
-					const uint32_t up = bd[k + 1];
-					const uint32_t cD = dg + (((nz[k >> 3] >> (4 * (k & 7) + 3)) & 1u) << SS), cU = up + STEP_U, cL = left + STEP_L;
-					uint32_t cm = cD < cU ? cD : cU;
-					cm = cm < cL ? cm : cL;
-					cm &= ~0x300u;
-					uint32_t cell = cm >= LIM ? INVALID : cm;
-					if (k > kmax) cell = INVALID;
-					bd[k] = cell;
-					left = cell;
-					dg = up;
-				}
-			} else {
-				uint32_t left = (x0 - 1 == 0) ? col0 : INVALID;
-				uint32_t dg = bd[0];
-				#pragma unroll
-				for (int k = 0; k < WB; ++k) {
-					const uint32_t r = (dd[k >> 3] >> (4 * (k & 7))) & 15u;
-					const uint32_t up = bd[k + 1];
-					const uint32_t cstS = ((mrow >> r) & 1u) ? 0u : (((m1 >> r) & 1u) ? (1u << SS) : (255u << SS));
-					const uint32_t cD = dg + cstS, cU = up + STEP_U, cL = left + STEP_L;
-					uint32_t cm = cD < cU ? cD : cU;
-					cm = cm < cL ? cm : cL;
-					cm &= ~0x300u;
-					uint32_t cell = cm >= LIM ? INVALID : cm;
-					if (x0 < 1) { const int x = x0 + k; if (x < 1) cell = x == 0 ? col0 : INVALID; }
-					if (k > kmax) cell = INVALID;
-					bd[k] = cell;
-					left = cell;
-					dg = up;
-				}
-			}
-			++p;
-			if ((p & 7) == 0) {
-				#pragma unroll
-				for (int i = 0; i < NW - 1; ++i) d[i] = d[i + 1];
-				d[NW - 1] = pick4(ahead, (uint32_t)jn & 3u);
-				dclean = all_acgt();
-				++j8; ++jn;
-				if ((jn & 3) == 0) ahead = ref_chunk_at(refw, rbase, jn >> 2, nchunks);
-			}
-		}
-		#pragma unroll
-		for (int k = 0; k < WB; ++k) {
-			const int x = (int)m + dlo + k;
-			if (k < Wd && x >= 1 && x <= (int)L) { const uint32_t key = bd[k] >> GS; if (key < bkey) { bkey = key; bv = bd[k] & 255u; } }
-		}
-		#pragma unroll
-		for (int k = 0; k < WB; ++k) {
-			const int x = (int)m + dlo + k;
-			if (k < Wd && x >= 1 && x <= (int)L && (bd[k] >> GS) == bkey) fin = (uint32_t)x;
-		}
+		const RefLaneAt ref{refw, hp->rbase, (L + 31) >> 5};
+		const BhipBandResult r = bhip_rescore_band<WB>(ref, qpack + (uint64_t)q * qw, qw, m, B, hp->e_first, hp->e_last, L, s_mm, fastq, rows8, nullptr);
+		bkey = r.bkey; bv = r.bv; fin = r.fin;
 	}
 	const uint32_t bs = bkey >> 8, bh = 255u - (bkey & 255u);
 	const bool ok = live && bs == B;
@@ -1323,16 +1222,22 @@
 template <int SET>
 __global__ __launch_bounds__(64) void k_rescore_reg(
 		const BhipRawHit *__restrict__ raw, const uint32_t *__restrict__ lists, const uint32_t *__restrict__ counts, uint32_t raw_cap,
-		const uint64_t *__restrict__ qoff, const uint8_t *__restrict__ qrc, const uint32_t *__restrict__ qpack, uint32_t qw,
-		const uint8_t *__restrict__ refb, const uint64_t *__restrict__ ref_off, const uint32_t *__restrict__ clump_len,
-		const uint8_t *__restrict__ lut,
+		const uint8_t *__restrict__ qrc, const uint32_t *__restrict__ qpack, uint32_t qw,
+		const uint8_t *__restrict__ refb, const uint32_t *__restrict__ mmtab, int rows8_opt,
 		BhipHit *__restrict__ out, uint32_t *__restrict__ n_out, uint32_t out_cap, uint32_t *__restrict__ err_flags) {
 	__shared__ uint32_t s_mm[16];
 	const uint32_t tid = threadIdx.x;
-	if (tid < 16) { uint32_t mm = 0; for (int r = 0; r < 16; ++r) mm |= (lut[16 * tid + r] == 0 ? 1u : 0u) << r | (lut[16 * tid + r] != 255 ? 1u : 0u) << (16 + r); s_mm[tid] = mm; }
+	{
+		constexpr int b0 = SET == 0 ? 0 : SET == 3 ? 3 : SET == 1 ? 4 : 6, b1 = SET == 0 ? 3 : SET == 3 ? 4 : SET == 1 ? 6 : 9;
+		uint32_t nmax = 0;
+		#pragma unroll
+		for (int b = b0; b < b1; ++b) nmax = counts[b] > nmax ? counts[b] : nmax;
+		if (blockIdx.x * 64u >= nmax) return;
+	}
+	if (tid < 16) s_mm[tid] = mmtab[tid];
 	__syncthreads();
-	uint32_t fastq = 0;
-	for (uint32_t qc = 1; qc <= 4; ++qc) if ((s_mm[qc] & 0x1Eu) == (1u << qc)) fastq |= 1u << qc;
+	const uint32_t fastq = mmtab[16];
+	const bool rows8 = rows8_opt && mmtab[17];
 	const uint32_t *refw = (const uint32_t *)refb;
 #define BHIP_RS_RUN(b, WB) { \
 		uint32_t n = counts[b]; if (n > raw_cap) n = raw_cap; \
@@ -1340,7 +1245,7 @@
 		const uint32_t n_round = (n + 63u) & ~63u; \
 		for (uint32_t i = blockIdx.x * 64 + tid; i < n_round; i += gridDim.x * 64) { \
 			const bool live = i < n; \
-			rescore_reg_one<WB>(raw + (live ? lst[i] : 0u), live, s_mm, fastq, tid, qoff, qrc, qpack, qw, refw, ref_off, clump_len, out, n_out, out_cap, err_flags); \
+			rescore_reg_one<WB>(raw + (live ? lst[i] : 0u), live, s_mm, fastq, rows8, tid, qrc, qpack, qw, refw, out, n_out, out_cap, err_flags); \
 		} }
 	if (SET == 0) { BHIP_RS_RUN(0, 4) BHIP_RS_RUN(1, 6) BHIP_RS_RUN(2, 8) }
 	else if (SET == 3) { BHIP_RS_RUN(3, 12) }
@@ -1348,14 +1253,14 @@
 	else { BHIP_RS_RUN(6, 32) BHIP_RS_RUN(7, 40) BHIP_RS_RUN(8, 48) }
 #undef BHIP_RS_RUN
 }
-template __global__ void k_rescore_reg<0>(const BhipRawHit *, const uint32_t *, const uint32_t *, uint32_t, const uint64_t *, const uint8_t *, const uint32_t *, uint32_t,
-	const uint8_t *, const uint64_t *, const uint32_t *, const uint8_t *, BhipHit *, uint32_t *, uint32_t, uint32_t *);
-template __global__ void k_rescore_reg<1>(const BhipRawHit *, const uint32_t *, const uint32_t *, uint32_t, const uint64_t *, const uint8_t *, const uint32_t *, uint32_t,
-	const uint8_t *, const uint64_t *, const uint32_t *, const uint8_t *, BhipHit *, uint32_t *, uint32_t, uint32_t *);
-template __global__ void k_rescore_reg<2>(const BhipRawHit *, const uint32_t *, const uint32_t *, uint32_t, const uint64_t *, const uint8_t *, const uint32_t *, uint32_t,
-	const uint8_t *, const uint64_t *, const uint32_t *, const uint8_t *, BhipHit *, uint32_t *, uint32_t, uint32_t *);
-template __global__ void k_rescore_reg<3>(const BhipRawHit *, const uint32_t *, const uint32_t *, uint32_t, const uint64_t *, const uint8_t *, const uint32_t *, uint32_t,
-	const uint8_t *, const uint64_t *, const uint32_t *, const uint8_t *, BhipHit *, uint32_t *, uint32_t, uint32_t *);
+template __global__ void k_rescore_reg<0>(const BhipRawHit *, const uint32_t *, const uint32_t *, uint32_t, const uint8_t *, const uint32_t *, uint32_t,
+	const uint8_t *, const uint32_t *, int, BhipHit *, uint32_t *, uint32_t, uint32_t *);
+template __global__ void k_rescore_reg<1>(const BhipRawHit *, const uint32_t *, const uint32_t *, uint32_t, const uint8_t *, const uint32_t *, uint32_t,
+	const uint8_t *, const uint32_t *, int, BhipHit *, uint32_t *, uint32_t, uint32_t *);
+template __global__ void k_rescore_reg<2>(const BhipRawHit *, const uint32_t *, const uint32_t *, uint32_t, const uint8_t *, const uint32_t *, uint32_t,
+	const uint8_t *, const uint32_t *, int, BhipHit *, uint32_t *, uint32_t, uint32_t *);
+template __global__ void k_rescore_reg<3>(const BhipRawHit *, const uint32_t *, const uint32_t *, uint32_t, const uint8_t *, const uint32_t *, uint32_t,
+	const uint8_t *, const uint32_t *, int, BhipHit *, uint32_t *, uint32_t, uint32_t *);
 
 template __global__ void k_rescore<false>(const BhipRawHit *, const uint32_t *, uint32_t, const uint32_t *, const uint32_t *, const uint32_t *, int,
 	const uint8_t *, const uint64_t *, const uint32_t *, const uint8_t *, const uint8_t *, const uint64_t *, const uint32_t *, const uint8_t *,
diff --git a/burst_amd/csrc/bhip_rescore_band.h b/burst_amd/csrc/bhip_rescore_band.h
--- /dev/null
+++ b/burst_amd/csrc/bhip_rescore_band.h
@@ -0,0 +1,207 @@
+#pragma once
+#include <stdint.h>
+#ifdef __HIPCC__
+#define BHIP_BAND_FN __device__ __forceinline__
+#define BHIP_BAND_UNROLL _Pragma("unroll")
+BHIP_BAND_FN uint32_t bhip_alignbit(uint32_t hi, uint32_t lo, uint32_t sh) { return __builtin_amdgcn_alignbit(hi, lo, sh); }
+#else
+#define BHIP_BAND_FN static inline
+#define BHIP_BAND_UNROLL
+#ifndef BHIP_HOST_UINT4
+#define BHIP_HOST_UINT4
+struct uint4 { uint32_t x, y, z, w; };
+#endif
+BHIP_BAND_FN uint32_t bhip_alignbit(uint32_t hi, uint32_t lo, uint32_t sh) { return (uint32_t)(((((uint64_t)hi) << 32) | lo) >> (sh & 31u)); }
+#endif
+
+#define BHIP_RS_MM_WORDS 18
+#define BHIP_RS_ROWS8_MAXWB 12
+
+static inline void bhip_rescore_masks(const uint8_t *lut, uint32_t out[BHIP_RS_MM_WORDS]) {
+	for (int q = 0; q < 16; ++q) {
+		uint32_t mm = 0;
+		for (int r = 0; r < 16; ++r) mm |= (lut[16 * q + r] == 0 ? 1u : 0u) << r | (lut[16 * q + r] != 255 ? 1u : 0u) << (16 + r);
+		out[q] = mm;
+	}
+	uint32_t fastq = 0, pad255 = 1;
+	for (uint32_t qc = 1; qc <= 4; ++qc) { if ((out[qc] & 0x1Eu) == (1u << qc)) fastq |= 1u << qc; if (lut[16 * qc] != 255) pad255 = 0; }
+	out[16] = fastq;
+	out[17] = fastq == 0x1Eu && pad255 ? 1u : 0u;
+}
+
+BHIP_BAND_FN uint32_t bhip_pick4(const uint4 v, uint32_t i) { return i == 0 ? v.x : i == 1 ? v.y : i == 2 ? v.z : v.w; }
+BHIP_BAND_FN bool bhip_dword_acgt(uint32_t d) { return ((d - 0x11111111u) & 0xCCCCCCCCu) == 0; }
+
+struct BhipBandResult { uint32_t bkey, bv, fin; };
+
+template <int WB> struct BhipBandWmin { static constexpr int value = WB == 4 ? 3 : WB == 6 ? 5 : WB == 8 ? 7 : WB == 12 ? 9 : 1; };
+
+template <int WB, class REF>
+BHIP_BAND_FN BhipBandResult bhip_rescore_band(const REF &ref, const uint32_t *qp, uint32_t qw, uint32_t m, uint32_t B,
+		uint32_t h_first, uint32_t h_last, uint32_t L, const uint32_t *mm, uint32_t fastq, bool rows8, uint32_t *stat) {
+	constexpr int NW = (WB + 7) / 8 + 1;
+	constexpr bool ROWS8 = WB <= BHIP_RS_ROWS8_MAXWB;
+	constexpr int WMIN = BhipBandWmin<WB>::value;
+	constexpr uint32_t SS = 18, GS = 10;
+	const uint32_t INVALID = (512u << SS) | (255u << GS), Z0 = 255u << GS;
+	const uint32_t STEP_U = (1u << SS) + 1u + (1u << 8), STEP_L = (1u << SS) - (1u << GS) + (2u << 8);
+	BhipBandResult res; res.bkey = 0xFFFFFFFFu; res.bv = 0; res.fin = 0xFFFFFFFFu;
+	const int e2 = (int)(h_last < L ? h_last : L), e1 = (int)h_first;
+	const int dlo = e1 - (int)m - (int)B, Wd = e2 - e1 + 2 * (int)B + 1;
+	const uint32_t LIM = (B + 1) << SS;
+	uint32_t bd[WB + 1];
+	BHIP_BAND_UNROLL
+	for (int k = 0; k < WB; ++k) { const int x = dlo + k; bd[k] = (k < Wd && x >= 0 && x <= (int)L) ? Z0 : INVALID; }
+	bd[WB] = INVALID;
+	int p = dlo, j8 = dlo >> 3;
+	uint32_t d[NW];
+	BHIP_BAND_UNROLL
+	for (int i = 0; i < NW; ++i) d[i] = ref.dword(j8 + i);
+	auto all_acgt = [&]() { uint32_t bad = 0;
+		BHIP_BAND_UNROLL
+		for (int i = 0; i < NW; ++i) bad |= (d[i] - 0x11111111u) & 0xCCCCCCCCu;
+		return bad == 0; };
+	bool dclean = all_acgt();
+	int jn = j8 + NW;
+	uint4 ahead = ref.chunk(jn >> 2);
+	uint32_t qd = qp[0], q_next = qw > 1 ? qp[1] : 0u;
+	uint32_t prev_sym = (ref.dword((p - 1) >> 3) >> (4 * ((p - 1) & 7))) & 15u;
+	int ylo = 9 > 1 - dlo ? 9 : 1 - dlo, yhi = (int)m - 7 < (int)L - Wd - 6 - dlo ? (int)m - 7 : (int)L - Wd - 6 - dlo;
+	if (!ROWS8 || !rows8 || B > 8u || Wd < WMIN) yhi = 0;
+	uint32_t limk[WB > WMIN ? WB - WMIN : 1];
+	BHIP_BAND_UNROLL
+	for (int k = WMIN; k < WB; ++k) limk[k - WMIN] = k < Wd ? LIM : 0u;
+	int y = 1;
+	while (y <= (int)m) {
+		const uint32_t qi = (uint32_t)(y - 1);
+		if ((qi & 7u) == 0 && qi) { qd = q_next; q_next = (qi >> 3) + 1 < qw ? qp[(qi >> 3) + 1] : 0u; }
+		if (ROWS8 && (qi & 7u) == 0 && y >= ylo && y <= yhi) {
+			const uint32_t dnext = bhip_pick4(ahead, (uint32_t)jn & 3u);
+			if (dclean && bhip_dword_acgt(dnext) && bhip_dword_acgt(qd)) {
+				uint32_t e[NW];
+				{
+					const uint32_t sh = 4u * ((uint32_t)p & 7u);
+					BHIP_BAND_UNROLL
+					for (int i = 0; i < NW - 1; ++i) e[i] = bhip_alignbit(d[i + 1], d[i], sh);
+					e[NW - 1] = bhip_alignbit(dnext, d[NW - 1], sh);
+				}
+				BHIP_BAND_UNROLL
+				for (int r = 0; r < 8; ++r) {
+					const uint32_t qx = ((qd >> (4 * r)) & 15u) * 0x11111111u;
+					uint32_t nz[NW];
+					BHIP_BAND_UNROLL
+					for (int i = 0; i < NW; ++i) { const uint32_t x = e[i] ^ qx; nz[i] = ((x & 0x77777777u) + 0x77777777u) | x; }
+					uint32_t left = INVALID;
+					uint32_t dg = bd[0];
+					BHIP_BAND_UNROLL
+					for (int k = 0; k < WB; ++k) {
+						const uint32_t up = bd[k + 1];
+						const uint32_t cD = dg + (((nz[(r + k) >> 3] >> (4 * ((r + k) & 7) + 3)) & 1u) << SS), cU = up + STEP_U, cL = left + STEP_L;
+						uint32_t cm = cD < cU ? cD : cU;
+						cm = cm < cL ? cm : cL;
+						cm &= ~0x300u;
+						const uint32_t cell = cm >= (k < WMIN ? LIM : limk[k < WMIN ? 0 : k - WMIN]) ? INVALID : cm;
+						bd[k] = cell;
+						left = cell;
+						dg = up;
+					}
+				}
+				BHIP_BAND_UNROLL
+				for (int i = 0; i < NW - 1; ++i) d[i] = d[i + 1];
+				d[NW - 1] = dnext;
+				p += 8; ++j8; ++jn;
+				if ((jn & 3) == 0) ahead = ref.chunk_clamped(jn >> 2);
+				y += 8;
+				if (stat) ++stat[0];
+				continue;
+			}
+		}
+		const uint32_t qc = (qd >> (4 * (qi & 7u))) & 15u;
+		const uint32_t col0 = (uint32_t)y <= B ? (((uint32_t)y << SS) | Z0 | (uint32_t)y) : INVALID;
+		const int x0 = y + dlo;
+		const bool fast_row = y > 1 && x0 >= 1 && dclean && ((fastq >> qc) & 1u);
+		const uint32_t mrow = fast_row ? 0u : mm[qc];
+		const uint32_t m1 = mrow >> 16;
+		uint32_t dd[NW - 1];
+		{
+			const uint32_t sh = 4u * ((uint32_t)p & 7u);
+			BHIP_BAND_UNROLL
+			for (int i = 0; i < NW - 1; ++i) dd[i] = bhip_alignbit(d[i + 1], d[i], sh);
+		}
+		const int kmax = (Wd - 1) < ((int)L - x0) ? (Wd - 1) : ((int)L - x0);
+		if (y == 1) {
+			BHIP_BAND_UNROLL
+			for (int k = 0; k < WB; ++k) {
+				const int x = x0 + k;
+				const uint32_t r = (dd[k >> 3] >> (4 * (k & 7))) & 15u;
+				const uint32_t cst = ((mrow >> r) & 1u) ? 0u : (((m1 >> r) & 1u) ? 1u : 255u);
+				uint32_t hh = 0;
+				if (cst == 1 && x >= 2) hh = (mrow >> prev_sym) & 1u;
+				uint32_t cell = cst == 255u ? INVALID : ((cst << SS) | ((255u - hh) << GS));
+				if (x < 1) cell = x == 0 ? col0 : INVALID;
+				if (k > kmax) cell = INVALID;
+				prev_sym = r;
+				bd[k] = cell;
+			}
+		} else if (fast_row) {
+			uint32_t nz[NW - 1];
+			BHIP_BAND_UNROLL
+			for (int i = 0; i < NW - 1; ++i) { const uint32_t x = dd[i] ^ (qc * 0x11111111u); nz[i] = ((x & 0x77777777u) + 0x77777777u) | x; }
+			uint32_t left = (x0 - 1 == 0) ? col0 : INVALID;
+			uint32_t dg = bd[0];
+			BHIP_BAND_UNROLL
+			for (int k = 0; k < WB; ++k) {
+				const uint32_t up = bd[k + 1];
+				const uint32_t cD = dg + (((nz[k >> 3] >> (4 * (k & 7) + 3)) & 1u) << SS), cU = up + STEP_U, cL = left + STEP_L;
+				uint32_t cm = cD < cU ? cD : cU;
+				cm = cm < cL ? cm : cL;
+				cm &= ~0x300u;
+				uint32_t cell = cm >= LIM ? INVALID : cm;
+				if (k > kmax) cell = INVALID;
+				bd[k] = cell;
+				left = cell;
+				dg = up;
+			}
+		} else {
+			uint32_t left = (x0 - 1 == 0) ? col0 : INVALID;
+			uint32_t dg = bd[0];
+			BHIP_BAND_UNROLL
+			for (int k = 0; k < WB; ++k) {
+				const uint32_t r = (dd[k >> 3] >> (4 * (k & 7))) & 15u;
+				const uint32_t up = bd[k + 1];
+				const uint32_t cstS = ((mrow >> r) & 1u) ? 0u : (((m1 >> r) & 1u) ? (1u << SS) : (255u << SS));
+				const uint32_t cD = dg + cstS, cU = up + STEP_U, cL = left + STEP_L;
+				uint32_t cm = cD < cU ? cD : cU;
+				cm = cm < cL ? cm : cL;
+				cm &= ~0x300u;
+				uint32_t cell = cm >= LIM ? INVALID : cm;
+				if (x0 < 1) { const int x = x0 + k; if (x < 1) cell = x == 0 ? col0 : INVALID; }
+				if (k > kmax) cell = INVALID;
+				bd[k] = cell;
+				left = cell;
+				dg = up;
+			}
+		}
+		++p;
+		if ((p & 7) == 0) {
+			BHIP_BAND_UNROLL
+			for (int i = 0; i < NW - 1; ++i) d[i] = d[i + 1];
+			d[NW - 1] = bhip_pick4(ahead, (uint32_t)jn & 3u);
+			dclean = all_acgt();
+			++j8; ++jn;
+			if ((jn & 3) == 0) ahead = ref.chunk(jn >> 2);
+		}
+		++y;
+	}
+	BHIP_BAND_UNROLL
+	for (int k = 0; k < WB; ++k) {
+		const int x = (int)m + dlo + k;
+		if (k < Wd && x >= 1 && x <= (int)L) { const uint32_t key = bd[k] >> GS; if (key < res.bkey) { res.bkey = key; res.bv = bd[k] & 255u; } }
+	}
+	BHIP_BAND_UNROLL
+	for (int k = 0; k < WB; ++k) {
+		const int x = (int)m + dlo + k;
+		if (k < Wd && x >= 1 && x <= (int)L && (bd[k] >> GS) == res.bkey) res.fin = (uint32_t)x;
+	}
+	return res;
+}
```

After: 582.5 million. -5.7%, worse.
